# zipnn/zipnn

Measured on NVIDIA H100. Metric: compress+decompress GB/s on bf16 tensors, higher is better.
Workload: dtype u8

## Files before the change

zipnn_b200/csrc/api_compress.inc:

```

namespace {
struct EncWs {
  size_t part_off, part_bytes, types_off, sizes_off, itemoff_off, saves_off, hist_off, total;
};
inline EncWs enc_ws_layout(size_t n, int G, size_t chunk) {
  EncWs L;
  const uint64_t nitems = (uint64_t)G * num_chunks(n, chunk);
  L.part_off = kCtrlBytes;
  L.part_bytes = 8 * (size_t)G * ((num_chunks(n, chunk) + kScanItems - 1) / kScanItems);
  L.types_off = round_up(L.part_off + L.part_bytes, 256);
  L.sizes_off = round_up(L.types_off + nitems, 256);
  L.itemoff_off = round_up(L.sizes_off + 4 * nitems, 256);
  L.saves_off = round_up(L.itemoff_off + 8 * nitems, 256);
  L.hist_off = round_up(L.saves_off + sizeof(EncSave) * nitems, 256);
  L.total = L.hist_off + 2048 * nitems + 256;
  return L;
}

template <int G>
int launch_encode(const uint8_t* in, size_t n, uint32_t chunk, uint64_t K, int bits_mode, double thr, uint8_t* ws,
                  const EncWs& L, const void* h_hdr, uint32_t hdr_len, uint8_t* out, cudaStream_t st, void* h_total = nullptr,
                  cudaEvent_t len_ready = nullptr) {
  Ctrl* ctrl = (Ctrl*)ws;
  uint8_t* types = ws + L.types_off;
  uint32_t* sizes = (uint32_t*)(ws + L.sizes_off);
  uint64_t* item_off = (uint64_t*)(ws + L.itemoff_off);
  EncSave* saves = (EncSave*)(ws + L.saves_off);
  const int sms = sm_count_cached();
  uint16_t* hist = (uint16_t*)(ws + L.hist_off);
  ZB_CUDA(cudaMemsetAsync(ws, 0, L.types_off, st));
  {
    const size_t smem = sizeof(HistSmem<G>);
    if (smem > 48 * 1024 && !smem_attr(k_encode_hist<G>, smem)) return ZIPNN_B200_E_CUDA;
    const int blocks = (int)std::min<uint64_t>(K, (uint64_t)sms * resident_blocks(k_encode_hist<G>, smem, kEncThreads));
    ScopedTimer tm(kKEncodeStats, st);
    k_encode_hist<G><<<blocks, kEncThreads, smem, st>>>(in, n, chunk, K, bits_mode, hist);
    ZB_LAUNCHED();
  }
  {
    const size_t smem = sizeof(TableWarp) * kTableWarps;
    const uint64_t nitems = (uint64_t)G * K;
    const int blocks = (int)std::min<uint64_t>((nitems + kTableWarps - 1) / kTableWarps, (uint64_t)sms * 16);
    ScopedTimer tm(kKEncodeTable, st);
    k_encode_table<G><<<blocks, kTableWarps * 32, smem, st>>>(hist, n, chunk, K, thr, types, sizes, saves,
                                                              (unsigned long long*)(ws + L.part_off));
    ZB_LAUNCHED();
  }
  {
    ScopedTimer tm(kKEncodeScan, st);
    const unsigned nblk = (unsigned)((K + kScanItems - 1) / kScanItems);
    EncHeader hdr;
    memcpy(hdr.b, h_hdr, hdr_len);
    k_encode_scan<<<(unsigned)G * nblk, kScanThreads, 0, st>>>(sizes, types, G, K, hdr, hdr_len, out, item_off, ctrl,
                                                            (const unsigned long long*)(ws + L.part_off));
    ZB_LAUNCHED();
  }
  if (h_total) {
    ZB_CUDA(cudaMemcpyAsync(h_total, &ctrl->total_len, sizeof(uint64_t), cudaMemcpyDeviceToHost, st));
    ZB_CUDA(cudaEventRecord(len_ready, st));
  }
  if (chunk % (64u * G) != 0) {
    const int blocks = (int)std::min<uint64_t>((uint64_t)G * K, (uint64_t)sms * resident_blocks(k_encode_write<G>, 0, kEncThreads));
    ScopedTimer tm(kKEncodeWriteRagged, st);
    k_encode_write<G><<<blocks, kEncThreads, 0, st>>>(in, n, chunk, K, bits_mode, types, sizes, saves, item_off, out, 0);
    ZB_LAUNCHED();
    return ZIPNN_B200_OK;
  }
  {
    const int blocks = (int)std::min<uint64_t>(K, (uint64_t)sms * resident_blocks(k_encode_write_warp<G>, 0, kWbWarps * 32));
    ScopedTimer tm(kKEncodeWrite, st);
    k_encode_write_warp<G><<<blocks, kWbWarps * 32, 0, st>>>(in, n, chunk, K, bits_mode, types, sizes, saves, item_off, out);
    ZB_LAUNCHED();
  }
  if ((n % chunk) % (64u * G) != 0) {
    ScopedTimer tm(kKEncodeWriteRagged, st);
    k_encode_write<G><<<G, kEncThreads, 0, st>>>(in, n, chunk, K, bits_mode, types, sizes, saves, item_off, out, 1);
    ZB_LAUNCHED();
  }
  return ZIPNN_B200_OK;
}
}

extern "C" int zipnn_b200_compress_workspace_size(size_t n, int num_buf, size_t chunk, size_t* out) {
  if (!out || chunk == 0 || !(num_buf == 1 || num_buf == 2 || num_buf == 4)) return ZIPNN_B200_E_ARG;
  *out = enc_ws_layout(n, num_buf, chunk).total;
  return ZIPNN_B200_OK;
}

extern "C" int zipnn_b200_compress(const void* d_in, size_t n, const void* h_hdr, size_t hdr_len, int num_buf, int bits_mode,
                        int bytes_mode, size_t chunk, float threshold, void* d_out, size_t out_cap, size_t* out_len,
                        void* d_ws, size_t ws_bytes, void* cuda_stream) {
  if (!valid_layout(num_buf, bytes_mode, chunk)) return ZIPNN_B200_E_ARG;
  if (!h_hdr || hdr_len < 32 || hdr_len > kHdrMax || !d_out || !d_ws) return ZIPNN_B200_E_ARG;
  if (n && (!d_in || ((uintptr_t)d_in & 15))) return ZIPNN_B200_E_ARG;
  if ((uintptr_t)d_ws & 255) return ZIPNN_B200_E_ARG;
  size_t bound = 0;
  zipnn_b200_compress_bound(n, num_buf, chunk, hdr_len, &bound);
  if (out_cap < bound) return ZIPNN_B200_E_CAPACITY;
  cudaStream_t st = (cudaStream_t)cuda_stream;
  if (n == 0) {
    uint8_t tmp[kHdrMax];
    memcpy(tmp, h_hdr, hdr_len);
    const uint64_t t = hdr_len;
    memcpy(tmp + 24, &t, 8);
    ZB_CUDA(cudaMemcpyAsync(d_out, tmp, hdr_len, cudaMemcpyHostToDevice, st));
    ZB_CUDA(cudaStreamSynchronize(st));
    if (out_len) *out_len = hdr_len;
    return ZIPNN_B200_OK;
  }
  const EncWs L = enc_ws_layout(n, num_buf, chunk);
  if (ws_bytes < L.total) return ZIPNN_B200_E_CAPACITY;
  uint8_t* ws = (uint8_t*)d_ws;
  const uint64_t K = num_chunks(n, chunk);
  const double thr = (double)threshold;
  PinnedBlock total;
  WaitEvent len_ready;
  if (out_len && (!total.p || !len_ready.e)) return ZIPNN_B200_E_CUDA;
  const int rc = dispatch_G(num_buf, [&](auto g) -> int {
    return launch_encode<decltype(g)::value>((const uint8_t*)d_in, n, (uint32_t)chunk, K, bits_mode, thr, ws, L, h_hdr,
                                             (uint32_t)hdr_len, (uint8_t*)d_out, st, out_len ? total.p : nullptr, len_ready.e);
  });
  if (out_len) {
    const bool ok = cuda_ok(cudaEventSynchronize(len_ready.e));
    if (rc) return rc;
    if (!ok) return ZIPNN_B200_E_CUDA;
    uint64_t v = 0;
    memcpy(&v, total.p, sizeof(v));
    *out_len = (size_t)v;
  }
  return rc;
}

namespace {
static_assert(sizeof(size_t) == sizeof(uint64_t), "out_lens are filled by a strided copy of Ctrl::total_len");
constexpr int kEncBatchKernels = 5;
constexpr uint64_t kEncBatchMaxChunks = 16384;

uint64_t enc_batch_max_chunks() {
  const char* e = getenv("ZIPNN_B200_ENC_BATCH_MAX_CHUNKS");
  return e ? (uint64_t)atoll(e) : kEncBatchMaxChunks;
}

int check_compress_item(const zipnn_b200_compress_item& it) {
  if (!valid_layout(it.num_buf, it.bytes_mode, it.chunk)) return ZIPNN_B200_E_ARG;
  if (!it.h_hdr || it.hdr_len < 32 || it.hdr_len > kHdrMax || !it.d_out) return ZIPNN_B200_E_ARG;
  if (it.n && (!it.d_in || ((uintptr_t)it.d_in & 15))) return ZIPNN_B200_E_ARG;
  size_t bound = 0;
  zipnn_b200_compress_bound(it.n, it.num_buf, it.chunk, it.hdr_len, &bound);
  if (it.out_cap < bound) return ZIPNN_B200_E_CAPACITY;
  return ZIPNN_B200_OK;
}

inline int enc_class(int G) { return G == 1 ? 0 : (G == 2 ? 1 : 2); }

struct EncBatchLayout {
  std::vector<int> order;
  int cls_begin[4] = {0, 0, 0, 0};
  std::vector<uint64_t> starts;
  size_t start_at[3] = {0, 0, 0};
  std::vector<size_t> hdr_at, part_at, slice_at;
  std::vector<int> single;
  std::vector<char> one;
  size_t start_off = 0, hdr_off = 0, blob_bytes = 0, ctrl_off = 0, zero_bytes = 0, total = 0;
};

int enc_batch_layout(const zipnn_b200_compress_item* items, int n, EncBatchLayout& L) {
  if (n < 0 || (n && !items)) return ZIPNN_B200_E_ARG;
  for (int k = 0; k < 3; k++) {
    L.cls_begin[k] = (int)L.order.size();
    for (int i = 0; i < n; i++) {
      if (!(items[i].num_buf == 1 || items[i].num_buf == 2 || items[i].num_buf == 4)) return ZIPNN_B200_E_ARG;
      if (enc_class(items[i].num_buf) == k) L.order.push_back(i);
    }
  }
  L.cls_begin[3] = n;
  L.hdr_at.resize(n);
  L.part_at.resize(n);
  L.slice_at.resize(n);
  const uint64_t max_chunks = enc_batch_max_chunks();
  auto is_single = [&](int i) { return num_chunks(items[i].n, items[i].chunk) > max_chunks; };
  L.one.resize(n);
  for (int i = 0; i < n; i++)
    if ((L.one[i] = is_single(i))) L.single.push_back(i);
  for (int k = 0; k < 3; k++) {
    const int b = L.cls_begin[k], m = L.cls_begin[k + 1] - b;
    L.start_at[k] = L.starts.size();
    L.starts.resize(L.starts.size() + (size_t)kEncBatchKernels * (m + 1), 0);
    uint64_t* s = L.starts.data() + L.start_at[k];
    for (int j = 0; j < m; j++) {
      const zipnn_b200_compress_item& it = items[L.order[b + j]];
      const uint64_t G = (uint64_t)it.num_buf, K = num_chunks(it.n, it.chunk);
      const bool one = is_single(L.order[b + j]);
      const uint64_t work[kEncBatchKernels] = {
          K, G * K, K ? G * ((K + kScanItems - 1) / kScanItems) : 1, it.chunk % (64 * G) == 0 ? K : 0,
          it.chunk % (64 * G) != 0 ? G * K : ((it.n % it.chunk) % (64 * G) != 0 ? G : 0)};
      for (int q = 0; q < kEncBatchKernels; q++) s[q * (m + 1) + j + 1] = s[q * (m + 1) + j] + (one ? 0 : work[q]);
    }
    if (s[2 * (m + 1) + m] > 0x7fffffffull) return ZIPNN_B200_E_ARG;
  }
  L.start_off = round_up(sizeof(EncTensor) * (size_t)n, 256);
  L.hdr_off = round_up(L.start_off + sizeof(uint64_t) * L.starts.size(), 256);
  size_t at = L.hdr_off;
  for (int i = 0; i < n; i++) {
    L.hdr_at[i] = at;
    at += round_up(items[i].hdr_len, 16);
  }
  L.blob_bytes = at;
  L.ctrl_off = round_up(at, 256);
  at = L.ctrl_off + kCtrlBytes * (size_t)n;
  for (int i = 0; i < n; i++) {
    L.part_at[i] = at;
    at += items[i].n ? enc_ws_layout(items[i].n, items[i].num_buf, items[i].chunk).part_bytes : 0;
  }
  L.zero_bytes = at - L.ctrl_off;
  at = round_up(at, 256);
  for (int i = 0; i < n; i++) {
    L.slice_at[i] = at;
    if (items[i].n) {
      const EncWs W = enc_ws_layout(items[i].n, items[i].num_buf, items[i].chunk);
      at += round_up(is_single(i) ? W.total : W.total - W.types_off, 256);
    }
  }
  L.total = at;
  return ZIPNN_B200_OK;
}

template <int G>
int launch_encode_batch(const EncTensor* d_t, uint32_t m, const uint64_t* d_start, const uint64_t* h_start, cudaStream_t st) {
  auto batch = [&](int q) { EncBatch b; b.t = d_t; b.start = d_start + (size_t)q * (m + 1); b.n = m; return b; };
  auto total = [&](int q) { return h_start[(size_t)q * (m + 1) + m]; };
  const int sms = sm_count_cached();
  {
    const size_t smem = sizeof(HistSmem<G>);
    if (smem > 48 * 1024 && !smem_attr(k_encode_hist_batch<G>, smem)) return ZIPNN_B200_E_CUDA;
    const int per_sm = resident_blocks(k_encode_hist_batch<G>, smem, kEncThreads);
    const int blocks = (int)std::max<uint64_t>(1, std::min<uint64_t>(total(0), (uint64_t)sms * per_sm));
    ScopedTimer tm(kKEncodeStats, st);
    k_encode_hist_batch<G><<<blocks, kEncThreads, smem, st>>>(batch(0));
    ZB_LAUNCHED();
  }
  {
    const size_t smem = sizeof(TableWarp) * kTableWarps;
    const int blocks = (int)std::max<uint64_t>(1, std::min<uint64_t>((total(1) + kTableWarps - 1) / kTableWarps, (uint64_t)sms * 16));
    ScopedTimer tm(kKEncodeTable, st);
    k_encode_table_batch<G><<<blocks, kTableWarps * 32, smem, st>>>(batch(1));
    ZB_LAUNCHED();
  }
  {
    ScopedTimer tm(kKEncodeScan, st);
    k_encode_scan_batch<<<(unsigned)total(2), kScanThreads, 0, st>>>(batch(2));
    ZB_LAUNCHED();
  }
  {
    const int per_sm = resident_blocks(k_encode_write_warp<G, EncBatch>, 0, kWbWarps * 32);
    const int blocks = (int)std::max<uint64_t>(1, std::min<uint64_t>(total(3), (uint64_t)sms * per_sm));
    ScopedTimer tm(kKEncodeWrite, st);
    k_encode_write_warp<G, EncBatch><<<blocks, kWbWarps * 32, 0, st>>>(nullptr, 0, 0, 0, 0, nullptr, nullptr, nullptr, nullptr, nullptr, batch(3));
    ZB_LAUNCHED();
  }
  if (total(4)) {
    const int per_sm = resident_blocks(k_encode_write<G, EncBatch>, 0, kEncThreads);
    const int blocks = (int)std::min<uint64_t>(total(4), (uint64_t)sms * per_sm);
    ScopedTimer tm(kKEncodeWriteRagged, st);
    k_encode_write<G, EncBatch><<<blocks, kEncThreads, 0, st>>>(nullptr, 0, 0, 0, 0, nullptr, nullptr, nullptr, nullptr, nullptr, 0, batch(4));
    ZB_LAUNCHED();
  }
  return ZIPNN_B200_OK;
}
}

extern "C" int zipnn_b200_compress_batch_workspace_size(const zipnn_b200_compress_item* items, int n, size_t* out) {
  if (!out) return ZIPNN_B200_E_ARG;
  for (int i = 0; i < n && items; i++)
    if (!valid_layout(items[i].num_buf, items[i].bytes_mode, items[i].chunk)) return ZIPNN_B200_E_ARG;
  EncBatchLayout L;
  const int rc = enc_batch_layout(items, n, L);
  if (rc) return rc;
  *out = L.total;
  return ZIPNN_B200_OK;
}

extern "C" int zipnn_b200_compress_batch(const zipnn_b200_compress_item* items, int n, size_t* out_lens, void* d_ws, size_t ws_bytes,
                                         void* cuda_stream) {
  if (n < 0 || (n && !items)) return ZIPNN_B200_E_ARG;
  if (n == 0) return ZIPNN_B200_OK;
  if (!d_ws || ((uintptr_t)d_ws & 255)) return ZIPNN_B200_E_ARG;
  for (int i = 0; i < n; i++) {
    const int rc = check_compress_item(items[i]);
    if (rc) return rc;
  }
  EncBatchLayout L;
  {
    const int rc = enc_batch_layout(items, n, L);
    if (rc) return rc;
  }
  if (ws_bytes < L.total) return ZIPNN_B200_E_CAPACITY;
  uint8_t* ws = (uint8_t*)d_ws;
  std::vector<uint8_t> blob(L.blob_bytes, 0);
  EncTensor* T = reinterpret_cast<EncTensor*>(blob.data());
  for (int j = 0; j < n; j++) {
    const int i = L.order[j];
    const zipnn_b200_compress_item& it = items[i];
    const EncWs W = enc_ws_layout(it.n, it.num_buf, it.chunk);
    auto slice = [&](size_t off) { return ws + L.slice_at[i] + (off - (L.one[i] ? 0 : W.types_off)); };
    EncTensor& t = T[j];
    t.in = (const uint8_t*)it.d_in;
    t.out = (uint8_t*)it.d_out;
    t.hdr = ws + L.hdr_at[i];
    t.n = it.n;
    t.K = num_chunks(it.n, it.chunk);
    t.chunk = (uint32_t)it.chunk;
    t.hdr_len = (uint32_t)it.hdr_len;
    t.G = it.num_buf;
    t.bits_mode = it.bits_mode;
    t.thr = (double)it.threshold;
    t.ctrl = (Ctrl*)(ws + L.ctrl_off + kCtrlBytes * (size_t)i);
    t.partials = (unsigned long long*)(ws + L.part_at[i]);
    t.types = slice(W.types_off);
    t.sizes = (uint32_t*)slice(W.sizes_off);
    t.item_off = (uint64_t*)slice(W.itemoff_off);
    t.saves = (EncSave*)slice(W.saves_off);
    t.hist = (uint16_t*)slice(W.hist_off);
    memcpy(blob.data() + L.hdr_at[i], it.h_hdr, it.hdr_len);
  }
  memcpy(blob.data() + L.start_off, L.starts.data(), sizeof(uint64_t) * L.starts.size());
  cudaStream_t st = (cudaStream_t)cuda_stream;
  ZB_CUDA(cudaMemsetAsync(ws + L.ctrl_off, 0, L.zero_bytes, st));
  ZB_CUDA(cudaMemcpyAsync(ws, blob.data(), blob.size(), cudaMemcpyHostToDevice, st));
  for (int k = 0; k < 3; k++) {
    const uint32_t m = (uint32_t)(L.cls_begin[k + 1] - L.cls_begin[k]);
    if (m == 0 || L.starts[L.start_at[k] + 2 * (m + 1) + m] == 0) continue;
    const EncTensor* d_t = (const EncTensor*)ws + L.cls_begin[k];
    const uint64_t* d_start = (const uint64_t*)(ws + L.start_off) + L.start_at[k];
    const uint64_t* h_start = L.starts.data() + L.start_at[k];
    const int rc = dispatch_G(1 << k, [&](auto g) -> int { return launch_encode_batch<decltype(g)::value>(d_t, m, d_start, h_start, st); });
    if (rc) return rc;
  }
  for (int i : L.single) {
    const zipnn_b200_compress_item& it = items[i];
    const EncWs W = enc_ws_layout(it.n, it.num_buf, it.chunk);
    uint8_t* sws = ws + L.slice_at[i];
    const int rc = dispatch_G(it.num_buf, [&](auto g) -> int {
      return launch_encode<decltype(g)::value>((const uint8_t*)it.d_in, it.n, (uint32_t)it.chunk, num_chunks(it.n, it.chunk), it.bits_mode,
                                               (double)it.threshold, sws, W, it.h_hdr, (uint32_t)it.hdr_len, (uint8_t*)it.d_out, st);
    });
    if (rc) return rc;
    ZB_CUDA(cudaMemcpyAsync(ws + L.ctrl_off + kCtrlBytes * (size_t)i + offsetof(Ctrl, total_len), sws + offsetof(Ctrl, total_len),
                            sizeof(uint64_t), cudaMemcpyDeviceToDevice, st));
  }
  if (out_lens) {
    ZB_CUDA(cudaMemcpy2DAsync(out_lens, sizeof(size_t), ws + L.ctrl_off + offsetof(Ctrl, total_len), kCtrlBytes, sizeof(uint64_t),
                              (size_t)n, cudaMemcpyDeviceToHost, st));
    ZB_CUDA(cudaStreamSynchronize(st));
  }
  return ZIPNN_B200_OK;
}
```

zipnn_b200/csrc/encode.cuh:

```cuda
#pragma once
#include "common.cuh"
#include "stage1.cuh"

#include <type_traits>

namespace zb {

struct EncSave {
  uint8_t nb[256];
  uint8_t hdr[128];
  uint32_t hsize;
  uint32_t sbytes[4];
  uint32_t lg;
  uint32_t pad[2];
};
static_assert(sizeof(EncSave) == 416, "EncSave layout");

constexpr int kEncThreads = 256;

struct EncTensor {
  const uint8_t* in;
  uint8_t* out;
  const uint8_t* hdr;
  uint64_t n, K;
  uint32_t chunk, hdr_len;
  int G, bits_mode;
  double thr;
  Ctrl* ctrl;
  unsigned long long* partials;
  uint8_t* types;
  uint32_t* sizes;
  uint64_t* item_off;
  EncSave* saves;
  uint16_t* hist;
};

struct EncBatch {
  const EncTensor* t;
  const uint64_t* start;
  uint32_t n;
};
struct NoBatch {};
template <class Batch>
constexpr bool kIsBatch = !std::is_same<Batch, NoBatch>::value;
__device__ __forceinline__ uint64_t batch_work(NoBatch, uint64_t single) { return single; }
__device__ __forceinline__ uint64_t batch_work(const EncBatch& B, uint64_t) { return B.start[B.n]; }

template <int G>
__device__ __forceinline__ uint32_t rot_byte_at(const uint8_t* __restrict__ in_c, uint32_t chunk_len, uint32_t rot_words,
                                                uint32_t pos) {
  const uint32_t wi = pos >> 2;
  if (wi >= rot_words) return in_c[pos];
  (void)chunk_len;
  const uint32_t w = rot_word<G>(__ldg(reinterpret_cast<const uint32_t*>(in_c) + wi));
  return (w >> (8 * (pos & 3))) & 0xFFu;
}

template <int G>
struct HistCfg {
  static constexpr int R = (G == 4) ? 16 : 32;
  static constexpr int kShift = (G == 4) ? 6 : 7;
};

template <int G>
struct HistSmem {
  uint32_t rep[G][256][HistCfg<G>::R];
};

template <int G, class Batch>
__device__ __forceinline__ void encode_hist(const uint8_t* __restrict__ in, uint64_t n, uint32_t chunk, uint64_t K, int bits_mode,
                                            uint16_t* __restrict__ hist, Batch B) {
  extern __shared__ __align__(1024) unsigned char smem_raw[];
  HistSmem<G>& S = *reinterpret_cast<HistSmem<G>*>(smem_raw);
  constexpr int R = HistCfg<G>::R;
  const int tid = threadIdx.x, lane = tid & 31;
  const uint32_t col_bytes = (uint32_t)(lane % R) * 4;
  unsigned char* const col_p = reinterpret_cast<unsigned char*>(&S.rep[0][0][0]) + col_bytes;
  for (int i = tid; i < G * 256 * R; i += kEncThreads) (&S.rep[0][0][0])[i] = 0;
  __syncthreads();
  for (uint64_t w = blockIdx.x; w < batch_work(B, K); w += gridDim.x) {
    uint64_t c = w;
    if constexpr (kIsBatch<Batch>) {
      const uint32_t i = batch_find(B.start, B.n, w);
      const EncTensor& T = B.t[i];
      in = T.in; n = T.n; chunk = T.chunk; K = T.K; bits_mode = T.bits_mode; hist = T.hist;
      c = w - B.start[i];
    }
    const uint8_t* in_c = in + c * (uint64_t)chunk;
    const uint32_t chunk_len = (c == K - 1) ? (uint32_t)(n - c * (uint64_t)chunk) : chunk;
    const uint32_t rot_words = (bits_mode == 1 && G > 1) ? (chunk_len >> 2) : 0;
    const bool fast = (chunk_len % 64u) == 0;
    for (int q = 0; q < 4; q++) {
      const uint32_t inc = (q & 1) ? 0x10000u : 1u;
      if (fast) {
        const uint32_t qbytes = chunk_len >> 2;
        const uint4* src = reinterpret_cast<const uint4*>(in_c + (uint64_t)q * qbytes);
        const uint32_t nvec = qbytes >> 4;
        uint4 v[4], nv[4];
#pragma unroll
        for (int k = 0; k < 4; k++) {
          const uint32_t u = k * kEncThreads + tid;
          nv[k] = (u < nvec) ? __ldg(src + u) : make_uint4(0, 0, 0, 0);
        }
        for (uint32_t u0 = 0; u0 < nvec; u0 += 4 * kEncThreads) {
#pragma unroll
          for (int k = 0; k < 4; k++) v[k] = nv[k];
#pragma unroll
          for (int k = 0; k < 4; k++) {
            const uint32_t u = u0 + (4 + k) * kEncThreads + tid;
            if (u < nvec) nv[k] = __ldg(src + u);
          }
#pragma unroll
          for (int k = 0; k < 4; k++) {
            if (u0 + k * kEncThreads + tid < nvec) {
              uint32_t w[4] = {v[k].x, v[k].y, v[k].z, v[k].w};
#pragma unroll
              for (int i = 0; i < 4; i++) {
                if (rot_words) w[i] = rot_word<G>(w[i]);
#pragma unroll
                for (int b = 0; b < 4; b++) {
                  const uint32_t byte = __byte_perm(w[i], 0u, 0x4440u | (uint32_t)b);
                  atomicAdd(reinterpret_cast<uint32_t*>(col_p + ((4 * i + b) % G) * (256 * R * 4) + byte * (uint32_t)(R * 4)), inc);
                }
              }
            }
          }
        }
      } else {
        for (int g = 0; g < G; g++) {
          const uint32_t pl = plane_len(chunk_len, G, g);
          const uint32_t seg = (pl + 3) >> 2;
          const uint32_t j0 = min(pl, (uint32_t)q * seg), j1 = (q == 3) ? pl : min(pl, j0 + seg);
          for (uint32_t j = j0 + tid; j < j1; j += kEncThreads)
            atomicAdd(&S.rep[g][rot_byte_at<G>(in_c, chunk_len, rot_words, j * G + g)][lane % R], inc);
        }
      }
      if ((q & 1) == 0) continue;
      __syncthreads();
      for (int g = 0; g < G; g++) {
        uint32_t sum = 0;
#pragma unroll
        for (int r = 0; r < R; r++) {
          const int rr = (r + tid) % R;
          sum += S.rep[g][tid][rr];
          S.rep[g][tid][rr] = 0;
        }
        uint16_t* h = hist + (((uint64_t)g * K + c) * 4 + (q - 1)) * 256 + tid;
        h[0] = (uint16_t)(sum & 0xFFFFu);
        h[256] = (uint16_t)(sum >> 16);
      }
      __syncthreads();
    }
  }
}

template <int G>
__global__ void __launch_bounds__(kEncThreads) k_encode_hist(const uint8_t* __restrict__ in, uint64_t n, uint32_t chunk,
                                                             uint64_t K, int bits_mode, uint16_t* __restrict__ hist) {
  encode_hist<G>(in, n, chunk, K, bits_mode, hist, NoBatch{});
}

template <int G>
__global__ void __launch_bounds__(kEncThreads, G == 1 ? 2 : 3) k_encode_hist_batch(EncBatch B) {
  encode_hist<G>(nullptr, 0, 0, 0, 0, nullptr, B);
}

constexpr uint64_t kScanItems = 2048;

struct __align__(16) TableWarp {
  uint32_t total[256];
  uint8_t nb[256];
  uint8_t nzsym[256];
  TreeScratch tree;
};
constexpr int kTableWarps = 4;

__device__ void warp_block_decision(TableWarp& S, const uint16_t* __restrict__ hist, uint32_t plen, uint32_t cap, double thr,
                                    uint8_t* type_out, uint32_t* size_out, EncSave* save) {
  const int lane = threadIdx.x & 31;
  uint32_t* total = S.total;
  uint32_t largest = 0;
  int max_sym = -1;
  for (int s = lane; s < 256; s += 32) {
    const uint32_t t = (uint32_t)__ldg(hist + s) + __ldg(hist + 256 + s) + __ldg(hist + 512 + s) + __ldg(hist + 768 + s);
    total[s] = t;
    largest = max(largest, t);
    if (t) max_sym = s;
  }
#pragma unroll
  for (int o = 16; o; o >>= 1) {
    largest = max(largest, __shfl_xor_sync(0xffffffffu, largest, o));
    max_sym = max(max_sym, __shfl_xor_sync(0xffffffffu, max_sym, o));
  }
  __syncwarp();
  uint32_t stored = 0;
  const int early = huf_early_out(largest, plen);
  if (early == 1) {
    stored = huf_block_decision(true, nullptr, 0, plen, cap, thr);
    if (stored && lane == 0) {
      save->hdr[0] = (uint8_t)max_sym;
      save->hsize = 0;
    }
  }
  if (early == 2) {
    TreeScratch& T = S.tree;
    uint8_t* nz = S.nzsym;
    int k = 0;
    for (int base = 0; base < 256; base += 32) {
      const int s = base + lane;
      const bool p = total[s] != 0;
      const uint32_t m = __ballot_sync(0xffffffffu, p);
      if (p) nz[k + __popc(m & ((1u << lane) - 1u))] = (uint8_t)s;
      k += __popc(m);
    }
    __syncwarp();
    for (int i = lane; i < k; i += 32) {
      const uint32_t c = total[nz[i]];
      int rank = 0;
      for (int j = 0; j < k; j++) {
        const uint32_t cj = total[nz[j]];
        rank += (cj > c) || (cj == c && j < i);
      }
      T.cnt[rank] = c;
      T.sym[rank] = nz[i];
    }
    __syncwarp();
    int lg = 0, hsize = -1;
    if (lane == 0) {
      const int want = fse_pick_log(kHufLogDefault, plen, (uint32_t)max_sym, 1);
      lg = huf_lengths_from_sorted(T, k - 1, want, S.nb);
      hsize = huf_write_table(T, S.nb, max_sym, lg);
    }
    lg = __shfl_sync(0xffffffffu, lg, 0);
    hsize = __shfl_sync(0xffffffffu, hsize, 0);
    __syncwarp();
    if (hsize > 0 && (uint32_t)hsize + 12 < plen) {
      uint32_t bits[4] = {0, 0, 0, 0};
      for (int s = lane; s <= max_sym; s += 32) {
        const uint32_t l = S.nb[s];
#pragma unroll
        for (int q = 0; q < 4; q++) bits[q] += (uint32_t)__ldg(hist + 256 * q + s) * l;
      }
#pragma unroll
      for (int q = 0; q < 4; q++)
#pragma unroll
        for (int o = 16; o; o >>= 1) bits[q] += __shfl_xor_sync(0xffffffffu, bits[q], o);
      stored = huf_block_decision(false, bits, hsize, plen, cap, thr);
      if (stored) {
        for (int s = lane; s < 256; s += 32) save->nb[s] = S.nb[s];
        for (int i = lane; i < hsize; i += 32) save->hdr[i] = T.hdr[i];
        if (lane == 0) {
          save->hsize = (uint32_t)hsize;
          save->lg = (uint32_t)lg;
#pragma unroll
          for (int q = 0; q < 4; q++) save->sbytes[q] = (bits[q] >> 3) + 1;
        }
      }
    }
  }
  if (lane == 0) {
    *type_out = stored ? 1 : 0;
    *size_out = stored ? stored : plen;
  }
}

template <int G>
__device__ __forceinline__ void encode_table_item(TableWarp& S, const uint16_t* __restrict__ hist, uint64_t n, uint32_t chunk, uint64_t K,
                                                  double thr, uint8_t* types, uint32_t* sizes, EncSave* saves,
                                                  unsigned long long* partials, const int lane, uint64_t item) {
  {
    const int g = (int)(item / K);
    const uint64_t c = item - (uint64_t)g * K;
    const uint32_t chunk_len = (c == K - 1) ? (uint32_t)(n - c * (uint64_t)chunk) : chunk;
    warp_block_decision(S, hist + item * 1024, plane_len(chunk_len, G, g), chunk, thr, types + item, sizes + item, saves + item);
    __syncwarp();
    if (lane == 0) atomicAdd(partials + (uint64_t)g * ((K + kScanItems - 1) / kScanItems) + c / kScanItems, (unsigned long long)sizes[item]);
  }
}

template <int G>
__global__ void __launch_bounds__(kTableWarps * 32) k_encode_table(const uint16_t* __restrict__ hist, uint64_t n, uint32_t chunk,
                                                                   uint64_t K, double thr, uint8_t* types, uint32_t* sizes,
                                                                   EncSave* saves, unsigned long long* partials) {
  extern __shared__ __align__(1024) unsigned char smem_raw[];
  TableWarp& S = reinterpret_cast<TableWarp*>(smem_raw)[threadIdx.x >> 5];
  const int lane = threadIdx.x & 31;
  const uint64_t nitems = (uint64_t)G * K;
  for (uint64_t item = (uint64_t)blockIdx.x * kTableWarps + (threadIdx.x >> 5); item < nitems;
       item += (uint64_t)gridDim.x * kTableWarps)
    encode_table_item<G>(S, hist, n, chunk, K, thr, types, sizes, saves, partials, lane, item);
}

constexpr int kScanThreads = 256;

__device__ __forceinline__ void encode_scan_block(const uint32_t* __restrict__ sizes, const uint8_t* __restrict__ types, int G, uint64_t K,
                                                  const uint8_t* __restrict__ hdr_dev, uint32_t hdr_len, uint8_t* out, uint64_t* item_off,
                                                  Ctrl* ctrl, const unsigned long long* __restrict__ partials, uint32_t bid) {
  __shared__ uint64_t warp_tot[kScanThreads / 32];
  __shared__ uint64_t red[kScanThreads / 32][3];
  const int tid = threadIdx.x, lane = tid & 31, warp = tid >> 5;
  const uint64_t nitems = (uint64_t)G * K;
  const uint64_t nblk = (K + kScanItems - 1) / kScanItems;
  const int g = (int)(bid / nblk);
  const uint64_t blk = bid - (uint64_t)g * nblk;
  uint64_t s_groups = 0, s_blocks = 0, s_all = 0;
  for (uint64_t i = tid; i < (uint64_t)G * nblk; i += kScanThreads) {
    const uint64_t v = partials[i];
    const uint64_t gi = i / nblk;
    s_all += v;
    if (gi < (uint64_t)g) s_groups += v;
    if (gi == (uint64_t)g && i - gi * nblk < blk) s_blocks += v;
  }
#pragma unroll
  for (int o = 16; o; o >>= 1) {
    s_groups += __shfl_xor_sync(0xffffffffu, s_groups, o);
    s_blocks += __shfl_xor_sync(0xffffffffu, s_blocks, o);
    s_all += __shfl_xor_sync(0xffffffffu, s_all, o);
  }
  if (lane == 0) { red[warp][0] = s_groups; red[warp][1] = s_blocks; red[warp][2] = s_all; }
  __syncthreads();
  s_groups = s_blocks = s_all = 0;
  for (int w = 0; w < kScanThreads / 32; w++) { s_groups += red[w][0]; s_blocks += red[w][1]; s_all += red[w][2]; }
  const uint64_t payload0 = (uint64_t)hdr_len + 9 * nitems;
  const uint64_t base = payload0 + s_groups;
  const uint64_t c_first = blk * kScanItems + (uint64_t)tid * 8;
  uint32_t v[8];
  uint64_t run = 0;
#pragma unroll
  for (int j = 0; j < 8; j++) {
    v[j] = (c_first + j < K) ? sizes[(uint64_t)g * K + c_first + j] : 0u;
    run += v[j];
  }
  uint64_t x = run;
#pragma unroll
  for (int o = 1; o < 32; o <<= 1) {
    const uint64_t y = __shfl_up_sync(0xffffffffu, x, o);
    if (lane >= o) x += y;
  }
  if (lane == 31) warp_tot[warp] = x;
  __syncthreads();
  uint64_t pre = s_blocks + x - run;
  for (int w = 0; w < warp; w++) pre += warp_tot[w];
  uint8_t* cum_out = out + hdr_len + nitems;
#pragma unroll
  for (int j = 0; j < 8; j++) {
    const uint64_t c = c_first + j;
    if (c < K) {
      const uint64_t i = (uint64_t)g * K + c;
      item_off[i] = base + pre;
      pre += v[j];
      st_u64_bytes(cum_out + 8 * i, pre);
      out[hdr_len + i] = types[i];
    }
  }
  if (blk == 0 && tid == 0) {
    ctrl->base[g] = base;
    uint64_t tot = 0;
    for (uint64_t j = 0; j < nblk; j++) tot += partials[(uint64_t)g * nblk + j];
    ctrl->group_total[g] = tot;
  }
  if (bid == 0) {
    const uint64_t total = payload0 + s_all;
    for (uint32_t i = tid; i < hdr_len; i += kScanThreads) {
      uint8_t b = hdr_dev[i];
      if (i >= 24 && i < 32) b = (uint8_t)(total >> (8 * (i - 24)));
      out[i] = b;
    }
    if (tid == 0) ctrl->total_len = total;
  }
}

constexpr size_t kHdrMax = 4096;
struct EncHeader {
  uint8_t b[kHdrMax];
};

__global__ void __launch_bounds__(kScanThreads) k_encode_scan(const uint32_t* __restrict__ sizes, const uint8_t* __restrict__ types,
                                                              int G, uint64_t K, const __grid_constant__ EncHeader hdr,
                                                              uint32_t hdr_len, uint8_t* out, uint64_t* item_off, Ctrl* ctrl,
                                                              const unsigned long long* __restrict__ partials) {
  encode_scan_block(sizes, types, G, K, hdr.b, hdr_len, out, item_off, ctrl, partials, blockIdx.x);
}

constexpr uint32_t kEncTile = kEncThreads * 16;
constexpr uint32_t kBitBufWords = (kEncTile * 11) / 32 + 8;

struct WriteSmem {
  __align__(16) uint8_t tile[kEncTile + 16];
  uint32_t bitbuf[kBitBufWords];
  uint32_t code[256];
  uint32_t warp_sum[kEncThreads / 32];
  EncSave save;
};

template <int G>
__device__ __forceinline__ void stage_tile(uint8_t* tile, const uint8_t* __restrict__ in_c, uint32_t chunk_len,
                                           uint32_t rot_words, int g, uint32_t p0, uint32_t cnt) {
  const int tid = threadIdx.x;
  const bool fast = ((p0 * G) % 16u) == 0 && (cnt % 16u) == 0 && ((p0 + cnt) * (uint32_t)G <= (chunk_len & ~3u));
  if (fast) {
    for (uint32_t u = tid; u < (cnt >> 4); u += kEncThreads) {
      const uint4* src = reinterpret_cast<const uint4*>(in_c + (uint64_t)(p0 + 16 * u) * G);
      uint32_t w[4 * G];
#pragma unroll
      for (int i = 0; i < G; i++) {
        const uint4 v = __ldg(src + i);
        w[4 * i] = v.x; w[4 * i + 1] = v.y; w[4 * i + 2] = v.z; w[4 * i + 3] = v.w;
      }
      if (rot_words) {
#pragma unroll
        for (int i = 0; i < 4 * G; i++) w[i] = rot_word<G>(w[i]);
      }
      uint4 pv[G];
      split16<G>(w, pv);
      uint4 mine = pv[0];
#pragma unroll
      for (int k = 1; k < G; k++)
        if (g == k) mine = pv[k];
      *reinterpret_cast<uint4*>(tile + 16 * u) = mine;
    }
  } else {
    for (uint32_t j = tid; j < cnt; j += kEncThreads)
      tile[j] = (uint8_t)rot_byte_at<G>(in_c, chunk_len, rot_words, (p0 + j) * G + g);
  }
}

__device__ __forceinline__ void tile_to_global(const uint8_t* tile, uint8_t* dst, uint32_t cnt) {
  const int tid = threadIdx.x;
  const uint32_t head = min(cnt, (uint32_t)((16 - ((uintptr_t)dst & 15)) & 15));
  if ((uint32_t)tid < head) dst[tid] = tile[tid];
  const uint32_t nvec = (cnt - head) >> 4;
  const uint32_t* t32 = reinterpret_cast<const uint32_t*>(tile);
  for (uint32_t v = tid; v < nvec; v += kEncThreads) {
    const uint32_t o = head + 16 * v;
    const uint32_t sh = (o & 3) * 8;
    const uint32_t* p = t32 + (o >> 2);
    const uint32_t a0 = p[0], a1 = p[1], a2 = p[2], a3 = p[3], a4 = p[4];
    *reinterpret_cast<uint4*>(dst + o) = make_uint4(__funnelshift_r(a0, a1, sh), __funnelshift_r(a1, a2, sh),
                                                    __funnelshift_r(a2, a3, sh), __funnelshift_r(a3, a4, sh));
  }
  const uint32_t done = head + 16 * nvec;
  if ((uint32_t)tid < cnt - done) dst[done + tid] = tile[done + tid];
}

template <bool kValHigh>
__device__ __forceinline__ void warp_build_codes(const uint8_t* nb, int lg, uint32_t* code) {
  const int lane = threadIdx.x & 31;
  uint32_t per_len[kHufLogMax + 1];
#pragma unroll
  for (int l = 0; l <= kHufLogMax; l++) per_len[l] = 0;
  for (int base = 0; base < 256; base += 32) {
    const int mine = nb[base + lane];
#pragma unroll
    for (int l = 1; l <= kHufLogMax; l++) per_len[l] += __popc(__ballot_sync(0xffffffffu, mine == l));
  }
  uint32_t start[kHufLogMax + 1];
  {
    uint32_t v = 0;
#pragma unroll
    for (int l = kHufLogMax; l >= 1; l--) {
      if (l <= lg) {
        start[l] = v;
        v = (v + per_len[l]) >> 1;
      } else {
        start[l] = 0;
      }
    }
  }
  for (int base = 0; base < 256; base += 32) {
    const int mine = nb[base + lane];
    uint32_t val = 0;
#pragma unroll
    for (int l = 1; l <= kHufLogMax; l++) {
      const uint32_t m = __ballot_sync(0xffffffffu, mine == l);
      if (mine == l) val = start[l] + __popc(m & ((1u << lane) - 1u));
      start[l] += __popc(m);
    }
    code[base + lane] = kValHigh ? ((val << 8) | (uint32_t)mine) : (val | ((uint32_t)mine << 16));
  }
}

template <int G, class Batch = NoBatch>
__global__ void __launch_bounds__(kEncThreads) k_encode_write(const uint8_t* __restrict__ in, uint64_t n, uint32_t chunk, uint64_t K,
                                                              int bits_mode, const uint8_t* __restrict__ types,
                                                              const uint32_t* __restrict__ sizes, const EncSave* __restrict__ saves,
                                                              const uint64_t* __restrict__ item_off, uint8_t* out,
                                                              int only_ragged, Batch B = {}) {
  __shared__ WriteSmem S;
  const int tid = threadIdx.x, lane = tid & 31, warp = tid >> 5;
  const uint64_t nitems = (uint64_t)G * K;
  const uint64_t first = only_ragged ? (uint64_t)blockIdx.x * K + (K - 1) : blockIdx.x;
  const uint64_t step = only_ragged ? nitems : gridDim.x;
  for (uint64_t w = first; w < batch_work(B, nitems); w += step) {
    uint64_t item = w;
    if constexpr (kIsBatch<Batch>) {
      const uint32_t i = batch_find(B.start, B.n, w);
      const EncTensor& T = B.t[i];
      in = T.in; n = T.n; chunk = T.chunk; K = T.K; bits_mode = T.bits_mode;
      types = T.types; sizes = T.sizes; saves = T.saves; item_off = T.item_off; out = T.out;
      const uint64_t j = w - B.start[i];
      item = (chunk % (64u * G) != 0) ? j : j * K + (K - 1);
    }
    const int g = (int)(item / K);
    const uint64_t c = item - (uint64_t)g * K;
    const uint8_t* in_c = in + c * (uint64_t)chunk;
    const uint32_t chunk_len = (c == K - 1) ? (uint32_t)(n - c * (uint64_t)chunk) : chunk;
    if (only_ragged && chunk_len % (64u * G) == 0) continue;
    const uint32_t rot_words = (bits_mode == 1 && G > 1) ? (chunk_len >> 2) : 0;
    const uint32_t plen = plane_len(chunk_len, G, g);
    uint8_t* dest = out + item_off[item];
    const uint8_t type = types[item];
    const uint32_t size = sizes[item];
    if (plen == 0) continue;
    __syncthreads();
    if (type == 0) {
      for (uint32_t p0 = 0; p0 < plen; p0 += kEncTile) {
        const uint32_t cnt = min(kEncTile, plen - p0);
        stage_tile<G>(S.tile, in_c, chunk_len, rot_words, g, p0, cnt);
        __syncthreads();
        tile_to_global(S.tile, dest + p0, cnt);
        __syncthreads();
      }
      continue;
    }
    if (size == 1) {
      if (tid == 0) dest[0] = saves[item].hdr[0];
      continue;
    }
    {
      const uint32_t* sv = reinterpret_cast<const uint32_t*>(saves + item);
      uint32_t* dv = reinterpret_cast<uint32_t*>(&S.save);
      for (int i = tid; i < (int)(sizeof(EncSave) / 4); i += kEncThreads) dv[i] = sv[i];
    }
    __syncthreads();
    const uint32_t hsize = S.save.hsize;
    if (warp == 0) warp_build_codes<false>(S.save.nb, (int)S.save.lg, S.code);
    if (warp == 1) {
      for (uint32_t i = lane; i < hsize; i += 32) dest[i] = S.save.hdr[i];
      if (lane < 3) {
        dest[hsize + 2 * lane] = (uint8_t)S.save.sbytes[lane];
        dest[hsize + 2 * lane + 1] = (uint8_t)(S.save.sbytes[lane] >> 8);
      }
    }
    __syncthreads();
    const uint32_t seg = (plen + 3) >> 2;
    uint32_t stream_at = hsize + 6;
    for (int i = 0; i < 4; i++) {
      const uint32_t s_begin = (uint32_t)i * seg;
      const uint32_t s_end = (i == 3) ? plen : s_begin + seg;
      uint8_t* gaddr = dest + stream_at;
      const uint32_t sbytes = S.save.sbytes[i];
      stream_at += sbytes;
      const uint32_t a = (uint32_t)((uintptr_t)gaddr & 3);
      uint32_t* gword = reinterpret_cast<uint32_t*>(gaddr - a);
      uint32_t B = 8 * a;
      uint32_t flushed = 0;
      for (uint32_t w = tid; w < kBitBufWords; w += kEncThreads) S.bitbuf[w] = 0;
      __syncthreads();
      for (uint32_t p1 = s_end; p1 > s_begin;) {
        const uint32_t p0 = (p1 - s_begin > kEncTile) ? p1 - kEncTile : s_begin;
        const uint32_t cnt = p1 - p0;
        stage_tile<G>(S.tile, in_c, chunk_len, rot_words, g, p0, cnt);
        __syncthreads();
        const uint32_t e0 = 16u * tid;
        const int nvalid = (int)min(16u, cnt > e0 ? cnt - e0 : 0u);
        uint64_t v[4] = {0, 0, 0, 0};
        uint32_t l[4] = {0, 0, 0, 0};
        if (nvalid == 16 && (cnt & 15u) == 0) {
          const uint4 q = *reinterpret_cast<const uint4*>(S.tile + (cnt - 16 - e0));
          const uint32_t wv[4] = {q.x, q.y, q.z, q.w};
#pragma unroll
          for (int k = 0; k < 16; k++) {
            const uint32_t sym = (wv[(15 - k) >> 2] >> (8 * ((15 - k) & 3))) & 0xFFu;
            const uint32_t cd = S.code[sym];
            v[k >> 2] |= (uint64_t)(cd & 0xFFFFu) << l[k >> 2];
            l[k >> 2] += cd >> 16;
          }
        } else {
          for (int k = 0; k < nvalid; k++) {
            const uint32_t cd = S.code[S.tile[cnt - 1 - (e0 + k)]];
            v[k >> 2] |= (uint64_t)(cd & 0xFFFFu) << l[k >> 2];
            l[k >> 2] += cd >> 16;
          }
        }
        const uint32_t mine = l[0] + l[1] + l[2] + l[3];
        uint32_t x = mine;
#pragma unroll
        for (int o = 1; o < 32; o <<= 1) {
          const uint32_t y = __shfl_up_sync(0xffffffffu, x, o);
          if (lane >= o) x += y;
        }
        if (lane == 31) S.warp_sum[warp] = x;
        __syncthreads();
        uint32_t pre = 0, tile_bits = 0;
#pragma unroll
        for (int w = 0; w < kEncThreads / 32; w++) {
          const uint32_t t = S.warp_sum[w];
          if (w < warp) pre += t;
          tile_bits += t;
        }
        uint32_t off = (B - 32 * flushed) + pre + x - mine;
#pragma unroll
        for (int r = 0; r < 4; r++) {
          if (l[r]) {
            const uint32_t sh = off & 31, wi = off >> 5;
            const uint32_t lo32 = (uint32_t)v[r], hi32 = (uint32_t)(v[r] >> 32);
            const uint32_t w0 = lo32 << sh;
            const uint32_t w1 = __funnelshift_l(lo32, hi32, sh);
            const uint32_t w2 = sh ? (hi32 >> (32 - sh)) : 0u;
            if (w0) atomicOr(&S.bitbuf[wi], w0);
            if (w1) atomicOr(&S.bitbuf[wi + 1], w1);
            if (w2) atomicOr(&S.bitbuf[wi + 2], w2);
            off += l[r];
          }
        }
        __syncthreads();
        B += tile_bits;
        const uint32_t complete = (B >> 5) - flushed;
        for (uint32_t w = tid; w < complete; w += kEncThreads) {
          const uint32_t val = S.bitbuf[w];
          if (flushed + w == 0 && a != 0) {
            for (uint32_t bb = a; bb < 4; bb++) gaddr[bb - a] = (uint8_t)(val >> (8 * bb));
          } else {
            gword[flushed + w] = val;
          }
        }
        const uint32_t carry = S.bitbuf[complete];
        __syncthreads();
        for (uint32_t w = tid; w <= complete + 1 && w < kBitBufWords; w += kEncThreads) S.bitbuf[w] = 0;
        __syncthreads();
        if (tid == 0) S.bitbuf[0] = carry;
        flushed += complete;
        p1 = p0;
        __syncthreads();
      }
      if (tid == 0) S.bitbuf[(B - 32 * flushed) >> 5] |= 1u << (B & 31);
      __syncthreads();
      {
        const uint32_t first_byte = max(4 * flushed, a);
        const uint32_t end_byte = a + sbytes;
        for (uint32_t bb = first_byte + tid; bb < end_byte; bb += kEncThreads) {
          const uint32_t rel = bb - 4 * flushed;
          gaddr[bb - a] = (uint8_t)(S.bitbuf[rel >> 2] >> (8 * (rel & 3)));
        }
      }
      __syncthreads();
    }
  }
}

constexpr int kWbWarps = 4;
constexpr uint32_t kWbTile = 512;
constexpr uint32_t kWbBitWords = (kWbTile * 11) / 32 + 4;

__device__ __forceinline__ void rotate_planes(uint32_t& lo, uint32_t& hi) {
  const uint32_t l = lo, h = hi;
  hi = ((h << 1) & 0xFEFEFEFEu) | ((l >> 7) & 0x01010101u);
  lo = (h & 0x80808080u) | (l & 0x7F7F7F7Fu);
}

struct WbItem {
  uint8_t* dest;
  uint32_t size;
  uint32_t hsize;
  uint32_t sbytes[4];
  uint32_t lg;
  uint32_t type;
};

template <int G>
struct WbSmem {
  uint32_t code[G][256];
  WbItem item[G];
  __align__(16) uint8_t nb[G][256];
  uint32_t bitbuf[kWbWarps][G][kWbBitWords];
  __align__(16) uint8_t stage[kWbWarps][kWbTile + 32];
};

struct WbStream {
  uint8_t* gaddr;
  uint32_t a;
  uint32_t B;
  uint32_t flushed;
};

__device__ __forceinline__ void wb_flush(uint32_t* bitbuf, WbStream& st, int lane) {
  uint32_t* gword = reinterpret_cast<uint32_t*>(st.gaddr - st.a);
  const uint32_t complete = (st.B >> 5) - st.flushed;
  const bool split_first = (st.flushed == 0 && st.a != 0);
  if (split_first && lane == 0 && complete > 0) {
    const uint32_t val = bitbuf[0];
    for (uint32_t bb = st.a; bb < 4; bb++) st.gaddr[bb - st.a] = (uint8_t)(val >> (8 * bb));
  }
  for (uint32_t w = lane; w < complete; w += 32) {
    const uint32_t val = bitbuf[w];
    bitbuf[w] = 0;
    if (!(split_first && w == 0)) gword[st.flushed + w] = val;
  }
  if (lane == 0 && complete > 0) {
    bitbuf[0] = bitbuf[complete];
    bitbuf[complete] = 0;
  }
  st.flushed += complete;
  __syncwarp();
}

template <int G, class Batch = NoBatch>
__global__ void __launch_bounds__(kWbWarps * 32) k_encode_write_warp(const uint8_t* __restrict__ in, uint64_t n, uint32_t chunk,
                                                                     uint64_t K, int bits_mode, const uint8_t* __restrict__ types,
                                                                     const uint32_t* __restrict__ sizes,
                                                                     const EncSave* __restrict__ saves,
                                                                     const uint64_t* __restrict__ item_off, uint8_t* out,
                                                                     Batch B = {}) {
  __shared__ WbSmem<G> S;
  const int tid = threadIdx.x, lane = tid & 31, warp = tid >> 5;
  for (uint64_t w = blockIdx.x; w < batch_work(B, K); w += gridDim.x) {
    uint64_t c = w;
    if constexpr (kIsBatch<Batch>) {
      const uint32_t i = batch_find(B.start, B.n, w);
      const EncTensor& T = B.t[i];
      in = T.in; n = T.n; chunk = T.chunk; K = T.K; bits_mode = T.bits_mode;
      types = T.types; sizes = T.sizes; saves = T.saves; item_off = T.item_off; out = T.out;
      c = w - B.start[i];
    }
    const uint32_t chunk_len = (c == K - 1) ? (uint32_t)(n - c * (uint64_t)chunk) : chunk;
    if (chunk_len % (64u * G) != 0) continue;
    const uint8_t* in_c = in + c * (uint64_t)chunk;
    const uint32_t plen = chunk_len / G;
    const uint32_t seg = plen >> 2;
    const bool rot = (bits_mode == 1 && G > 1);
    __syncthreads();
    if (warp < G) {
      const int g = warp;
      const uint64_t item = (uint64_t)g * K + c;
      WbItem it;
      it.dest = out + item_off[item];
      it.type = types[item];
      it.size = sizes[item];
      it.hsize = 0;
      it.lg = 0;
      it.sbytes[0] = it.sbytes[1] = it.sbytes[2] = it.sbytes[3] = 0;
      if (it.type == 1 && it.size == 1) {
        if (lane == 0) it.dest[0] = saves[item].hdr[0];
      } else if (it.type == 1) {
        const EncSave* sv = saves + item;
        it.hsize = sv->hsize;
        it.lg = sv->lg;
#pragma unroll
        for (int q = 0; q < 4; q++) it.sbytes[q] = sv->sbytes[q];
        reinterpret_cast<uint2*>(S.nb[g])[lane] = reinterpret_cast<const uint2*>(sv->nb)[lane];
        __syncwarp();
        warp_build_codes<true>(S.nb[g], (int)it.lg, S.code[g]);
        for (uint32_t i = lane; i < it.hsize; i += 32) it.dest[i] = sv->hdr[i];
        if (lane < 3) {
          it.dest[it.hsize + 2 * lane] = (uint8_t)it.sbytes[lane];
          it.dest[it.hsize + 2 * lane + 1] = (uint8_t)(it.sbytes[lane] >> 8);
        }
      }
      if (lane == 0) S.item[g] = it;
    }
    __syncthreads();

    const int s = warp;
    WbStream st[G];
    uint32_t raw_shift[G];
#pragma unroll
    for (int g = 0; g < G; g++) {
      const WbItem& it = S.item[g];
      st[g].gaddr = it.dest;
      st[g].a = st[g].B = st[g].flushed = 0;
      raw_shift[g] = 0;
      if (it.type == 1 && it.size > 1) {
        uint32_t at = it.hsize + 6;
        for (int q = 0; q < s; q++) at += it.sbytes[q];
        st[g].gaddr = it.dest + at;
        st[g].a = (uint32_t)((uintptr_t)st[g].gaddr & 3);
        st[g].B = 8 * st[g].a;
        for (uint32_t w = lane; w < kWbBitWords; w += 32) S.bitbuf[warp][g][w] = 0;
      } else if (it.type == 0) {
        st[g].gaddr = it.dest + (uint64_t)s * seg;
        raw_shift[g] = (uint32_t)((uintptr_t)st[g].gaddr & 15);
      }
    }
    __syncwarp();

    const uint8_t* src_s = in_c + (uint64_t)s * seg * G;
    const uint32_t ntiles = (seg + kWbTile - 1) / kWbTile;
    uint4 cur[G], nxt[G];
    {
      const uint32_t t0 = (ntiles - 1) * kWbTile;
      if (t0 + 16 * lane < seg) {
        const uint4* p = reinterpret_cast<const uint4*>(src_s + (uint64_t)(t0 + 16 * lane) * G);
#pragma unroll
        for (int i = 0; i < G; i++) nxt[i] = __ldg(p + i);
      }
    }
    auto do_tile = [&](auto full_tag, const uint32_t ti) {
      constexpr bool kFull = decltype(full_tag)::value;
      const uint32_t t0 = ti * kWbTile;
      const uint32_t cnt = kFull ? kWbTile : min(kWbTile, seg - t0);
      const bool have = kFull ? true : (16u * lane < cnt);
#pragma unroll
      for (int i = 0; i < G; i++) cur[i] = nxt[i];
      if (ti > 0) {
        const uint4* p = reinterpret_cast<const uint4*>(src_s + (uint64_t)(t0 - kWbTile + 16 * lane) * G);
#pragma unroll
        for (int i = 0; i < G; i++) nxt[i] = __ldg(p + i);
      }
      uint4 pv[G];
      if (have) {
        uint32_t w[4 * G];
#pragma unroll
        for (int i = 0; i < G; i++) {
          w[4 * i] = cur[i].x; w[4 * i + 1] = cur[i].y; w[4 * i + 2] = cur[i].z; w[4 * i + 3] = cur[i].w;
        }
        split16<G>(w, pv);
        if (rot) {
          rotate_planes(pv[(G - 2) % G].x, pv[G - 1].x);
          rotate_planes(pv[(G - 2) % G].y, pv[G - 1].y);
          rotate_planes(pv[(G - 2) % G].z, pv[G - 1].z);
          rotate_planes(pv[(G - 2) % G].w, pv[G - 1].w);
        }
      }
#pragma unroll
      for (int g = 0; g < G; g++) {
        const uint32_t type = S.item[g].type, size = S.item[g].size;
        if (type == 0) {
          uint8_t* stg = S.stage[warp];
          if (have) *reinterpret_cast<uint4*>(stg + 16 * lane) = pv[g];
          __syncwarp();
          uint8_t* D = st[g].gaddr + t0;
          const uint32_t m = raw_shift[g];
          if (m == 0) {
            if (have) *reinterpret_cast<uint4*>(D + 16 * lane) = pv[g];
          } else {
            const uint32_t head = 16 - m;
            const uint32_t nblk = (cnt - head) >> 4;
            {
              const uint4 a4 = *reinterpret_cast<const uint4*>(stg + 16 * lane);
              const uint4 b4 = *reinterpret_cast<const uint4*>(stg + 16 * lane + 16);
              const uint32_t wv[8] = {a4.x, a4.y, a4.z, a4.w, b4.x, b4.y, b4.z, b4.w};
              const uint32_t bs = (head & 3) * 8;
              uint32_t o[4];
              switch (head >> 2) {
                case 0:
#pragma unroll
                  for (int i = 0; i < 4; i++) o[i] = __funnelshift_r(wv[i], wv[i + 1], bs);
                  break;
                case 1:
#pragma unroll
                  for (int i = 0; i < 4; i++) o[i] = __funnelshift_r(wv[i + 1], wv[i + 2], bs);
                  break;
                case 2:
#pragma unroll
                  for (int i = 0; i < 4; i++) o[i] = __funnelshift_r(wv[i + 2], wv[i + 3], bs);
                  break;
                default:
#pragma unroll
                  for (int i = 0; i < 4; i++) o[i] = __funnelshift_r(wv[i + 3], wv[i + 4], bs);
                  break;
              }
              if ((uint32_t)lane < nblk) *reinterpret_cast<uint4*>(D + head + 16 * lane) = make_uint4(o[0], o[1], o[2], o[3]);
            }
            if (kFull) {
              if (lane < 16) {
                const uint32_t idx = (uint32_t)lane < head ? (uint32_t)lane : (kWbTile - 16u + (uint32_t)lane);
                D[idx] = stg[idx];
              }
            } else {
              if ((uint32_t)lane < head) D[lane] = stg[lane];
              const uint32_t done = head + 16 * nblk;
              if ((uint32_t)lane < cnt - done) D[done + lane] = stg[done + lane];
            }
          }
          __syncwarp();
        } else if (size > 1) {
          const unsigned char* code = reinterpret_cast<const unsigned char*>(S.code[g]);
          uint64_t v[4] = {0, 0, 0, 0};
          uint32_t l[4] = {0, 0, 0, 0};
          if (have) {
            const uint32_t wv[4] = {pv[g].x, pv[g].y, pv[g].z, pv[g].w};
#pragma unroll
            for (int r = 0; r < 4; r++) {
              const uint32_t w = wv[3 - r];
              const uint32_t e3 = *reinterpret_cast<const uint32_t*>(code + ((w >> 22) & 0x3FCu));
              const uint32_t e2 = *reinterpret_cast<const uint32_t*>(code + ((w >> 14) & 0x3FCu));
              const uint32_t e1 = *reinterpret_cast<const uint32_t*>(code + ((w >> 6) & 0x3FCu));
              const uint32_t e0 = *reinterpret_cast<const uint32_t*>(code + ((w << 2) & 0x3FCu));
              const uint32_t n3 = e3 & 0xFFu, n2 = e2 & 0xFFu, n1 = e1 & 0xFFu, n0 = e0 & 0xFFu;
              const uint32_t hi = (e3 >> 8) | ((e2 >> 8) << n3);
              const uint32_t lo = (e1 >> 8) | ((e0 >> 8) << n1);
              const uint32_t lh = n3 + n2;
              v[r] = (uint64_t)hi | ((uint64_t)lo << lh);
              l[r] = lh + n1 + n0;
            }
          }
          const uint32_t mine = l[0] + l[1] + l[2] + l[3];
          uint32_t x = mine;
#pragma unroll
          for (int o = 1; o < 32; o <<= 1) {
            const uint32_t y = __shfl_down_sync(0xffffffffu, x, o);
            if (lane + o < 32) x += y;
          }
          const uint32_t tile_bits = __shfl_sync(0xffffffffu, x, 0);
          uint32_t* bitbuf = S.bitbuf[warp][g];
          uint32_t off = (st[g].B - 32 * st[g].flushed) + (x - mine);
          const uint32_t bitbuf_s = (uint32_t)__cvta_generic_to_shared(bitbuf);
#pragma unroll
          for (int r = 0; r < 4; r++) {
            const uint32_t sh = off & 31, sa = bitbuf_s + ((off >> 5) << 2);
            const uint32_t lo32 = (uint32_t)v[r], hi32 = (uint32_t)(v[r] >> 32);
            const uint32_t w0 = lo32 << sh;
            const uint32_t w1 = __funnelshift_l(lo32, hi32, sh);
            const uint32_t w2 = (hi32 >> 1) >> (31 - sh);
            asm volatile("red.shared.or.b32 [%0], %1;" ::"r"(sa), "r"(w0) : "memory");
            asm volatile("red.shared.or.b32 [%0+4], %1;" ::"r"(sa), "r"(w1) : "memory");
            asm volatile("{ .reg .pred p; setp.ne.u32 p, %1, 0; @p red.shared.or.b32 [%0+8], %1; }" ::"r"(sa), "r"(w2) : "memory");
            off += l[r];
          }
          __syncwarp();
          st[g].B += tile_bits;
          wb_flush(bitbuf, st[g], lane);
        }
      }
        };
    do_tile(std::false_type{}, ntiles - 1);
    for (uint32_t ti = ntiles - 1; ti-- > 0;) do_tile(std::true_type{}, ti);
#pragma unroll
    for (int g = 0; g < G; g++) {
      if (S.item[g].type == 1 && S.item[g].size > 1) {
        uint32_t* bitbuf = S.bitbuf[warp][g];
        if (lane == 0) bitbuf[(st[g].B - 32 * st[g].flushed) >> 5] |= 1u << (st[g].B & 31);
        __syncwarp();
        const uint32_t first_byte = max(4 * st[g].flushed, st[g].a);
        const uint32_t end_byte = st[g].a + S.item[g].sbytes[s];
        for (uint32_t bb = first_byte + lane; bb < end_byte; bb += 32) {
          const uint32_t rel = bb - 4 * st[g].flushed;
          st[g].gaddr[bb - st[g].a] = (uint8_t)(bitbuf[rel >> 2] >> (8 * (rel & 3)));
        }
        __syncwarp();
      }
    }
  }
}

template <int G>
__global__ void __launch_bounds__(kTableWarps * 32) k_encode_table_batch(EncBatch B) {
  extern __shared__ __align__(1024) unsigned char smem_raw[];
  TableWarp& S = reinterpret_cast<TableWarp*>(smem_raw)[threadIdx.x >> 5];
  const int lane = threadIdx.x & 31;
  const uint64_t total = B.start[B.n];
  for (uint64_t w = (uint64_t)blockIdx.x * kTableWarps + (threadIdx.x >> 5); w < total; w += (uint64_t)gridDim.x * kTableWarps) {
    const uint32_t i = batch_find(B.start, B.n, w);
    const EncTensor& T = B.t[i];
    encode_table_item<G>(S, T.hist, T.n, T.chunk, T.K, T.thr, T.types, T.sizes, T.saves, T.partials, lane, w - B.start[i]);
  }
}

__global__ void __launch_bounds__(kScanThreads) k_encode_scan_batch(EncBatch B) {
  const uint32_t i = batch_find(B.start, B.n, blockIdx.x);
  const EncTensor& T = B.t[i];
  if (T.K == 0) {
    for (uint32_t j = threadIdx.x; j < T.hdr_len; j += kScanThreads)
      T.out[j] = (j >= 24 && j < 32) ? (uint8_t)((uint64_t)T.hdr_len >> (8 * (j - 24))) : T.hdr[j];
    if (threadIdx.x == 0) T.ctrl->total_len = T.hdr_len;
    return;
  }
  encode_scan_block(T.sizes, T.types, T.G, T.K, T.hdr, T.hdr_len, T.out, T.item_off, T.ctrl, T.partials,
                    (uint32_t)(blockIdx.x - B.start[i]));
}

}
```

Before: 544.5.

## Prebuild Huffman codes in table pass and pipeline warp write with dynamic claims

Builds canonical Huffman code words once in the table kernel and stores them in EncSave, so the write kernels no longer rebuild codes per item. Moves the header and stream-size emission into the scan kernel. Restructures the warp write kernel into per-warp units claimed through an atomic work counter, double-buffering unit metadata and codes with cp.async so the next unit's fetch overlaps the current unit's coding. Adds an optional phase-timing and emit-ceiling probe under a compile flag. In exchange EncSave grows from 416 to 1184 bytes per item, and the per-warp double-buffered shared memory can lower occupancy.

```diff
diff --git a/zipnn_b200/csrc/api_compress.inc b/zipnn_b200/csrc/api_compress.inc
--- a/zipnn_b200/csrc/api_compress.inc
+++ b/zipnn_b200/csrc/api_compress.inc
@@ -51,7 +51,7 @@
     const unsigned nblk = (unsigned)((K + kScanItems - 1) / kScanItems);
     EncHeader hdr;
     memcpy(hdr.b, h_hdr, hdr_len);
-    k_encode_scan<<<(unsigned)G * nblk, kScanThreads, 0, st>>>(sizes, types, G, K, hdr, hdr_len, out, item_off, ctrl,
+    k_encode_scan<<<(unsigned)G * nblk, kScanThreads, 0, st>>>(sizes, types, saves, G, K, hdr, hdr_len, out, item_off, ctrl,
                                                             (const unsigned long long*)(ws + L.part_off));
     ZB_LAUNCHED();
   }
@@ -69,7 +69,8 @@
   {
     const int blocks = (int)std::min<uint64_t>(K, (uint64_t)sms * resident_blocks(k_encode_write_warp<G>, 0, kWbWarps * 32));
     ScopedTimer tm(kKEncodeWrite, st);
-    k_encode_write_warp<G><<<blocks, kWbWarps * 32, 0, st>>>(in, n, chunk, K, bits_mode, types, sizes, saves, item_off, out);
+    k_encode_write_warp<G><<<blocks, kWbWarps * 32, 0, st>>>(in, n, chunk, K, bits_mode, types, sizes, saves, item_off, out,
+                                                               &ctrl->work_counter);
     ZB_LAUNCHED();
   }
   if ((n % chunk) % (64u * G) != 0) {
@@ -255,7 +256,7 @@
     const int per_sm = resident_blocks(k_encode_write_warp<G, EncBatch>, 0, kWbWarps * 32);
     const int blocks = (int)std::max<uint64_t>(1, std::min<uint64_t>(total(3), (uint64_t)sms * per_sm));
     ScopedTimer tm(kKEncodeWrite, st);
-    k_encode_write_warp<G, EncBatch><<<blocks, kWbWarps * 32, 0, st>>>(nullptr, 0, 0, 0, 0, nullptr, nullptr, nullptr, nullptr, nullptr, batch(3));
+    k_encode_write_warp<G, EncBatch><<<blocks, kWbWarps * 32, 0, st>>>(nullptr, 0, 0, 0, 0, nullptr, nullptr, nullptr, nullptr, nullptr, nullptr, batch(3));
     ZB_LAUNCHED();
   }
   if (total(4)) {
@@ -355,3 +356,34 @@
   }
   return ZIPNN_B200_OK;
 }
+
+#ifdef ZB_EMIT_PHASES
+extern "C" int zipnn_b200_emit_phases_read(unsigned long long* out, int reset) {
+  if (!out) return ZIPNN_B200_E_ARG;
+  ZB_CUDA(cudaMemcpyFromSymbol(out, g_emit_phases, sizeof(g_emit_phases)));
+  if (reset) {
+    const unsigned long long zero[kPhCount] = {};
+    ZB_CUDA(cudaMemcpyToSymbol(g_emit_phases, zero, sizeof(zero)));
+  }
+  return ZIPNN_B200_OK;
+}
+
+extern "C" int zipnn_b200_emit_ceiling(const void* d_in, size_t n, int num_buf, size_t chunk, void* d_ws, void* d_out, void* cuda_stream) {
+  if (!d_in || !d_ws || !d_out || n == 0 || !(num_buf == 1 || num_buf == 2 || num_buf == 4) || chunk % (64u * num_buf) != 0)
+    return ZIPNN_B200_E_ARG;
+  const EncWs L = enc_ws_layout(n, num_buf, chunk);
+  uint8_t* ws = (uint8_t*)d_ws;
+  uint32_t* claim = &((Ctrl*)ws)->work_counter;
+  const uint64_t K = num_chunks(n, chunk);
+  cudaStream_t st = (cudaStream_t)cuda_stream;
+  ZB_CUDA(cudaMemsetAsync(claim, 0, sizeof(uint32_t), st));
+  return dispatch_G(num_buf, [&](auto g) -> int {
+    constexpr int G = decltype(g)::value;
+    const int blocks = (int)std::min<uint64_t>(K, (uint64_t)sm_count_cached() * resident_blocks(k_encode_write_warp<G>, 0, kWbWarps * 32));
+    k_emit_ceiling<G><<<blocks, kWbWarps * 32, 0, st>>>((const uint8_t*)d_in, n, (uint32_t)chunk, K, (const uint32_t*)(ws + L.sizes_off),
+                                                        (const uint64_t*)(ws + L.itemoff_off), (uint8_t*)d_out, claim);
+    ZB_CUDA(cudaGetLastError());
+    return ZIPNN_B200_OK;
+  });
+}
+#endif
diff --git a/zipnn_b200/csrc/encode.cuh b/zipnn_b200/csrc/encode.cuh
--- a/zipnn_b200/csrc/encode.cuh
+++ b/zipnn_b200/csrc/encode.cuh
@@ -2,19 +2,21 @@
 #include "common.cuh"
 #include "stage1.cuh"
 
+#include <cstddef>
 #include <type_traits>
 
 namespace zb {
 
 struct EncSave {
-  uint8_t nb[256];
+  uint32_t code[256];
   uint8_t hdr[128];
+  uint32_t sbytes[4];
   uint32_t hsize;
-  uint32_t sbytes[4];
-  uint32_t lg;
-  uint32_t pad[2];
-};
-static_assert(sizeof(EncSave) == 416, "EncSave layout");
+  uint32_t pad[3];
+};
+static_assert(sizeof(EncSave) == 1184 && sizeof(EncSave) % 16 == 0, "EncSave layout");
+static_assert(offsetof(EncSave, code) == 0 && offsetof(EncSave, hdr) == 1024 && offsetof(EncSave, sbytes) == 1152 &&
+              offsetof(EncSave, hsize) == 1168, "EncSave layout: code and sbytes are copied in 16-byte pieces");
 
 constexpr int kEncThreads = 256;
 
@@ -175,6 +177,42 @@
 };
 constexpr int kTableWarps = 4;
 
+__device__ __forceinline__ void warp_build_codes(const uint8_t* nb, int lg, uint32_t* code) {
+  const int lane = threadIdx.x & 31;
+  uint32_t per_len[kHufLogMax + 1];
+#pragma unroll
+  for (int l = 0; l <= kHufLogMax; l++) per_len[l] = 0;
+  for (int base = 0; base < 256; base += 32) {
+    const int mine = nb[base + lane];
+#pragma unroll
+    for (int l = 1; l <= kHufLogMax; l++) per_len[l] += __popc(__ballot_sync(0xffffffffu, mine == l));
+  }
+  uint32_t start[kHufLogMax + 1];
+  {
+    uint32_t v = 0;
+#pragma unroll
+    for (int l = kHufLogMax; l >= 1; l--) {
+      if (l <= lg) {
+        start[l] = v;
+        v = (v + per_len[l]) >> 1;
+      } else {
+        start[l] = 0;
+      }
+    }
+  }
+  for (int base = 0; base < 256; base += 32) {
+    const int mine = nb[base + lane];
+    uint32_t val = 0;
+#pragma unroll
+    for (int l = 1; l <= kHufLogMax; l++) {
+      const uint32_t m = __ballot_sync(0xffffffffu, mine == l);
+      if (mine == l) val = start[l] + __popc(m & ((1u << lane) - 1u));
+      start[l] += __popc(m);
+    }
+    code[base + lane] = (val << 8) | (uint32_t)mine;
+  }
+}
+
 __device__ void warp_block_decision(TableWarp& S, const uint16_t* __restrict__ hist, uint32_t plen, uint32_t cap, double thr,
                                     uint8_t* type_out, uint32_t* size_out, EncSave* save) {
   const int lane = threadIdx.x & 31;
@@ -247,11 +285,10 @@
         for (int o = 16; o; o >>= 1) bits[q] += __shfl_xor_sync(0xffffffffu, bits[q], o);
       stored = huf_block_decision(false, bits, hsize, plen, cap, thr);
       if (stored) {
-        for (int s = lane; s < 256; s += 32) save->nb[s] = S.nb[s];
+        warp_build_codes(S.nb, lg, save->code);
         for (int i = lane; i < hsize; i += 32) save->hdr[i] = T.hdr[i];
         if (lane == 0) {
           save->hsize = (uint32_t)hsize;
-          save->lg = (uint32_t)lg;
 #pragma unroll
           for (int q = 0; q < 4; q++) save->sbytes[q] = (bits[q] >> 3) + 1;
         }
@@ -293,7 +330,8 @@
 
 constexpr int kScanThreads = 256;
 
-__device__ __forceinline__ void encode_scan_block(const uint32_t* __restrict__ sizes, const uint8_t* __restrict__ types, int G, uint64_t K,
+__device__ __forceinline__ void encode_scan_block(const uint32_t* __restrict__ sizes, const uint8_t* __restrict__ types,
+                                                  const EncSave* __restrict__ saves, int G, uint64_t K,
                                                   const uint8_t* __restrict__ hdr_dev, uint32_t hdr_len, uint8_t* out, uint64_t* item_off,
                                                   Ctrl* ctrl, const unsigned long long* __restrict__ partials, uint32_t bid) {
   __shared__ uint64_t warp_tot[kScanThreads / 32];
@@ -353,6 +391,47 @@
       out[hdr_len + i] = types[i];
     }
   }
+  __syncthreads();
+  {
+    const uint64_t c_hi = min(K, (blk + 1) * kScanItems);
+    for (uint64_t c0 = blk * kScanItems + (uint64_t)warp * 16; c0 < c_hi; c0 += (kScanThreads / 32) * 16) {
+      const uint64_t i0 = (uint64_t)g * K + c0;
+      const uint32_t nk = (uint32_t)min((uint64_t)16, c_hi - c0);
+      uint32_t ty = 0, sz = 0, hs = 0, sb[3] = {0, 0, 0};
+      uint64_t off = 0;
+      if ((uint32_t)lane < nk) {
+        const uint64_t i = i0 + lane;
+        ty = types[i];
+        sz = sizes[i];
+        off = item_off[i];
+        hs = saves[i].hsize;
+#pragma unroll
+        for (int q = 0; q < 3; q++) sb[q] = saves[i].sbytes[q];
+      }
+      uint32_t hw[16];
+#pragma unroll
+      for (int k = 0; k < 16; k++) hw[k] = ((uint32_t)k < nk) ? reinterpret_cast<const uint32_t*>(saves[i0 + k].hdr)[lane] : 0u;
+#pragma unroll
+      for (int k = 0; k < 16; k++) {
+        const uint32_t t = __shfl_sync(0xffffffffu, ty, k), z = __shfl_sync(0xffffffffu, sz, k);
+        const uint32_t h = __shfl_sync(0xffffffffu, hs, k);
+        const uint32_t j0 = __shfl_sync(0xffffffffu, sb[0], k), j1 = __shfl_sync(0xffffffffu, sb[1], k);
+        const uint32_t j2 = __shfl_sync(0xffffffffu, sb[2], k);
+        const uint32_t jump = lane < 2 ? j0 : (lane < 4 ? j1 : j2);
+        const uint64_t o = __shfl_sync(0xffffffffu, off, k);
+        if ((uint32_t)k >= nk || t != 1) continue;
+        uint8_t* d = out + o;
+        if (z == 1) {
+          if (lane == 0) d[0] = (uint8_t)hw[k];
+          continue;
+        }
+#pragma unroll
+        for (int b = 0; b < 4; b++)
+          if (4u * lane + b < h) d[4 * lane + b] = (uint8_t)(hw[k] >> (8 * b));
+        if (lane < 6) d[h + lane] = (uint8_t)(jump >> (8 * (lane & 1)));
+      }
+    }
+  }
   if (blk == 0 && tid == 0) {
     ctrl->base[g] = base;
     uint64_t tot = 0;
@@ -376,10 +455,10 @@
 };
 
 __global__ void __launch_bounds__(kScanThreads) k_encode_scan(const uint32_t* __restrict__ sizes, const uint8_t* __restrict__ types,
-                                                              int G, uint64_t K, const __grid_constant__ EncHeader hdr,
+                                                              const EncSave* __restrict__ saves, int G, uint64_t K, const __grid_constant__ EncHeader hdr,
                                                               uint32_t hdr_len, uint8_t* out, uint64_t* item_off, Ctrl* ctrl,
                                                               const unsigned long long* __restrict__ partials) {
-  encode_scan_block(sizes, types, G, K, hdr.b, hdr_len, out, item_off, ctrl, partials, blockIdx.x);
+  encode_scan_block(sizes, types, saves, G, K, hdr.b, hdr_len, out, item_off, ctrl, partials, blockIdx.x);
 }
 
 constexpr uint32_t kEncTile = kEncThreads * 16;
@@ -390,8 +469,10 @@
   uint32_t bitbuf[kBitBufWords];
   uint32_t code[256];
   uint32_t warp_sum[kEncThreads / 32];
-  EncSave save;
-};
+  uint32_t sbytes[4];
+  uint32_t hsize;
+};
+static_assert(kEncThreads == 256, "k_encode_write: one code word per thread");
 
 template <int G>
 __device__ __forceinline__ void stage_tile(uint8_t* tile, const uint8_t* __restrict__ in_c, uint32_t chunk_len,
@@ -441,43 +522,6 @@
   }
   const uint32_t done = head + 16 * nvec;
   if ((uint32_t)tid < cnt - done) dst[done + tid] = tile[done + tid];
-}
-
-template <bool kValHigh>
-__device__ __forceinline__ void warp_build_codes(const uint8_t* nb, int lg, uint32_t* code) {
-  const int lane = threadIdx.x & 31;
-  uint32_t per_len[kHufLogMax + 1];
-#pragma unroll
-  for (int l = 0; l <= kHufLogMax; l++) per_len[l] = 0;
-  for (int base = 0; base < 256; base += 32) {
-    const int mine = nb[base + lane];
-#pragma unroll
-    for (int l = 1; l <= kHufLogMax; l++) per_len[l] += __popc(__ballot_sync(0xffffffffu, mine == l));
-  }
-  uint32_t start[kHufLogMax + 1];
-  {
-    uint32_t v = 0;
-#pragma unroll
-    for (int l = kHufLogMax; l >= 1; l--) {
-      if (l <= lg) {
-        start[l] = v;
-        v = (v + per_len[l]) >> 1;
-      } else {
-        start[l] = 0;
-      }
-    }
-  }
-  for (int base = 0; base < 256; base += 32) {
-    const int mine = nb[base + lane];
-    uint32_t val = 0;
-#pragma unroll
-    for (int l = 1; l <= kHufLogMax; l++) {
-      const uint32_t m = __ballot_sync(0xffffffffu, mine == l);
-      if (mine == l) val = start[l] + __popc(m & ((1u << lane) - 1u));
-      start[l] += __popc(m);
-    }
-    code[base + lane] = kValHigh ? ((val << 8) | (uint32_t)mine) : (val | ((uint32_t)mine << 16));
-  }
 }
 
 template <int G, class Batch = NoBatch>
@@ -523,33 +567,23 @@
       }
       continue;
     }
-    if (size == 1) {
-      if (tid == 0) dest[0] = saves[item].hdr[0];
-      continue;
-    }
+    if (size == 1) continue;
     {
-      const uint32_t* sv = reinterpret_cast<const uint32_t*>(saves + item);
-      uint32_t* dv = reinterpret_cast<uint32_t*>(&S.save);
-      for (int i = tid; i < (int)(sizeof(EncSave) / 4); i += kEncThreads) dv[i] = sv[i];
+      const EncSave& sv = saves[item];
+      const uint32_t e = sv.code[tid];
+      S.code[tid] = (e >> 8) | ((e & 0xFFu) << 16);
+      if (tid < 4) S.sbytes[tid] = sv.sbytes[tid];
+      if (tid == 0) S.hsize = sv.hsize;
     }
     __syncthreads();
-    const uint32_t hsize = S.save.hsize;
-    if (warp == 0) warp_build_codes<false>(S.save.nb, (int)S.save.lg, S.code);
-    if (warp == 1) {
-      for (uint32_t i = lane; i < hsize; i += 32) dest[i] = S.save.hdr[i];
-      if (lane < 3) {
-        dest[hsize + 2 * lane] = (uint8_t)S.save.sbytes[lane];
-        dest[hsize + 2 * lane + 1] = (uint8_t)(S.save.sbytes[lane] >> 8);
-      }
-    }
-    __syncthreads();
+    const uint32_t hsize = S.hsize;
     const uint32_t seg = (plen + 3) >> 2;
     uint32_t stream_at = hsize + 6;
     for (int i = 0; i < 4; i++) {
       const uint32_t s_begin = (uint32_t)i * seg;
       const uint32_t s_end = (i == 3) ? plen : s_begin + seg;
       uint8_t* gaddr = dest + stream_at;
-      const uint32_t sbytes = S.save.sbytes[i];
+      const uint32_t sbytes = S.sbytes[i];
       stream_at += sbytes;
       const uint32_t a = (uint32_t)((uintptr_t)gaddr & 3);
       uint32_t* gword = reinterpret_cast<uint32_t*>(gaddr - a);
@@ -659,23 +693,85 @@
   lo = (h & 0x80808080u) | (l & 0x7F7F7F7Fu);
 }
 
-struct WbItem {
-  uint8_t* dest;
-  uint32_t size;
-  uint32_t hsize;
-  uint32_t sbytes[4];
-  uint32_t lg;
-  uint32_t type;
+enum : uint32_t { kWbRaw = 0, kWbCoded = 1, kWbNone = 2 };
+
+template <int G>
+struct WbUnit {
+  const uint8_t* src;
+  uint8_t* dest[G];
+  uint32_t kind[G];
+  uint32_t sbytes[G];
+  uint32_t seg;
+  uint32_t rot;
+};
+
+struct __align__(16) WbFetch {
+  uint32_t sbytes[4][4];
+  uint64_t off[4];
+  uint32_t size[4];
+  uint32_t type4[4];
+  uint32_t hsize[4];
+  uint8_t* out;
+  const EncSave* save_c;
+  uint64_t K;
+  uint32_t item0;
+  uint32_t s;
 };
 
 template <int G>
 struct WbSmem {
-  uint32_t code[G][256];
-  WbItem item[G];
-  __align__(16) uint8_t nb[G][256];
+  uint32_t code[kWbWarps][2][G][256];
+  WbUnit<G> unit[kWbWarps][2];
+  WbFetch fetch[kWbWarps];
   uint32_t bitbuf[kWbWarps][G][kWbBitWords];
   __align__(16) uint8_t stage[kWbWarps][kWbTile + 32];
 };
+
+__device__ __forceinline__ void wb_cp_async(void* smem_dst, const void* gmem_src, int bytes) {
+  const uint32_t d = (uint32_t)__cvta_generic_to_shared(smem_dst);
+  if (bytes == 16) asm volatile("cp.async.cg.shared.global [%0], [%1], 16;\n" ::"r"(d), "l"(gmem_src) : "memory");
+  else if (bytes == 8) asm volatile("cp.async.ca.shared.global [%0], [%1], 8;\n" ::"r"(d), "l"(gmem_src) : "memory");
+  else asm volatile("cp.async.ca.shared.global [%0], [%1], 4;\n" ::"r"(d), "l"(gmem_src) : "memory");
+}
+__device__ __forceinline__ void wb_cp_async_wait() {
+  asm volatile("cp.async.commit_group;\ncp.async.wait_group 0;\n" ::: "memory");
+}
+
+enum : int { kPhSetup = 0, kPhWait = 1, kPhCode = 2, kPhTail = 3, kPhCount = 4 };
+#ifdef ZB_EMIT_PHASES
+__device__ unsigned long long g_emit_phases[kPhCount];
+struct PhaseClock {
+  long long last, acc[kPhCount];
+  __device__ __forceinline__ PhaseClock() {
+    last = clock64();
+#pragma unroll
+    for (int p = 0; p < kPhCount; p++) acc[p] = 0;
+  }
+  __device__ __forceinline__ void mark(int p) {
+    const long long t = clock64();
+    acc[p] += t - last;
+    last = t;
+  }
+  template <int N>
+  __device__ __forceinline__ void wait_for(const uint4 (&v)[N]) {
+#pragma unroll
+    for (int i = 0; i < N; i++) asm volatile("" ::"r"(v[i].x));
+    mark(kPhWait);
+  }
+  __device__ __forceinline__ void commit(int lane) {
+    if (lane == 0)
+#pragma unroll
+      for (int p = 0; p < kPhCount; p++) atomicAdd(&g_emit_phases[p], (unsigned long long)acc[p]);
+  }
+};
+#else
+struct PhaseClock {
+  __device__ __forceinline__ void mark(int) {}
+  template <int N>
+  __device__ __forceinline__ void wait_for(const uint4 (&)[N]) {}
+  __device__ __forceinline__ void commit(int) {}
+};
+#endif
 
 struct WbStream {
   uint8_t* gaddr;
@@ -705,16 +801,13 @@
   __syncwarp();
 }
 
-template <int G, class Batch = NoBatch>
-__global__ void __launch_bounds__(kWbWarps * 32) k_encode_write_warp(const uint8_t* __restrict__ in, uint64_t n, uint32_t chunk,
-                                                                     uint64_t K, int bits_mode, const uint8_t* __restrict__ types,
-                                                                     const uint32_t* __restrict__ sizes,
-                                                                     const EncSave* __restrict__ saves,
-                                                                     const uint64_t* __restrict__ item_off, uint8_t* out,
-                                                                     Batch B = {}) {
-  __shared__ WbSmem<G> S;
-  const int tid = threadIdx.x, lane = tid & 31, warp = tid >> 5;
-  for (uint64_t w = blockIdx.x; w < batch_work(B, K); w += gridDim.x) {
+template <int G, class Batch>
+__device__ __forceinline__ void wb_fetch_items(WbUnit<G>& U, WbFetch& F, uint64_t u, uint64_t units, const uint8_t* in, uint64_t n,
+                                               uint32_t chunk, uint64_t K, int bits_mode, const uint8_t* types, const uint32_t* sizes,
+                                               const EncSave* saves, const uint64_t* item_off, uint8_t* out, const Batch& B, int lane) {
+  uint32_t seg = 0;
+  if (u < units) {
+    const uint64_t w = u >> 2;
     uint64_t c = w;
     if constexpr (kIsBatch<Batch>) {
       const uint32_t i = batch_find(B.start, B.n, w);
@@ -724,77 +817,140 @@
       c = w - B.start[i];
     }
     const uint32_t chunk_len = (c == K - 1) ? (uint32_t)(n - c * (uint64_t)chunk) : chunk;
-    if (chunk_len % (64u * G) != 0) continue;
-    const uint8_t* in_c = in + c * (uint64_t)chunk;
-    const uint32_t plen = chunk_len / G;
-    const uint32_t seg = plen >> 2;
-    const bool rot = (bits_mode == 1 && G > 1);
-    __syncthreads();
-    if (warp < G) {
-      const int g = warp;
-      const uint64_t item = (uint64_t)g * K + c;
-      WbItem it;
-      it.dest = out + item_off[item];
-      it.type = types[item];
-      it.size = sizes[item];
-      it.hsize = 0;
-      it.lg = 0;
-      it.sbytes[0] = it.sbytes[1] = it.sbytes[2] = it.sbytes[3] = 0;
-      if (it.type == 1 && it.size == 1) {
-        if (lane == 0) it.dest[0] = saves[item].hdr[0];
-      } else if (it.type == 1) {
-        const EncSave* sv = saves + item;
-        it.hsize = sv->hsize;
-        it.lg = sv->lg;
-#pragma unroll
-        for (int q = 0; q < 4; q++) it.sbytes[q] = sv->sbytes[q];
-        reinterpret_cast<uint2*>(S.nb[g])[lane] = reinterpret_cast<const uint2*>(sv->nb)[lane];
-        __syncwarp();
-        warp_build_codes<true>(S.nb[g], (int)it.lg, S.code[g]);
-        for (uint32_t i = lane; i < it.hsize; i += 32) it.dest[i] = sv->hdr[i];
-        if (lane < 3) {
-          it.dest[it.hsize + 2 * lane] = (uint8_t)it.sbytes[lane];
-          it.dest[it.hsize + 2 * lane + 1] = (uint8_t)(it.sbytes[lane] >> 8);
-        }
-      }
-      if (lane == 0) S.item[g] = it;
-    }
-    __syncthreads();
-
-    const int s = warp;
+    if (chunk_len % (64u * G) == 0) {
+      const uint32_t s = (uint32_t)(u & 3);
+      seg = chunk_len / G / 4;
+      if (lane == 0) {
+        U.src = in + c * (uint64_t)chunk + (uint64_t)s * seg * G;
+        U.rot = (bits_mode == 1 && G > 1);
+        F.out = out;
+        F.save_c = saves + c;
+        F.K = K;
+        F.item0 = (uint32_t)(c & 3);
+        F.s = s;
+      }
+      const int g = lane & 7;
+      if (g < G) {
+        const uint64_t item = (uint64_t)g * K + c;
+        switch (lane >> 3) {
+          case 0: wb_cp_async(&F.off[g], item_off + item, 8); break;
+          case 1: wb_cp_async(&F.size[g], sizes + item, 4); break;
+          case 2: wb_cp_async(&F.type4[g], types + (item & ~(uint64_t)3), 4); break;
+          default:
+            wb_cp_async(F.sbytes[g], saves[item].sbytes, 16);
+            wb_cp_async(&F.hsize[g], &saves[item].hsize, 4);
+            break;
+        }
+      }
+    }
+  }
+  if (lane == 0) {
+    U.seg = seg;
+    if (seg == 0)
+#pragma unroll
+      for (int g = 0; g < G; g++) U.kind[g] = kWbNone;
+  }
+}
+
+template <int G>
+__device__ __forceinline__ void wb_fetch_codes(WbUnit<G>& U, const WbFetch& F, uint32_t (*code)[256], int lane) {
+  wb_cp_async_wait();
+  __syncwarp();
+  const uint32_t seg = U.seg;
+  if (seg == 0) return;
+#pragma unroll
+  for (int g = 0; g < G; g++) {
+    const uint64_t item_lo = (uint64_t)g * F.K + F.item0;
+    const uint32_t type = (F.type4[g] >> (8 * (uint32_t)(item_lo & 3))) & 0xFFu;
+    const uint32_t kind = type == 0 ? kWbRaw : (F.size[g] > 1 ? kWbCoded : kWbNone);
+    uint8_t* dest = F.out + F.off[g];
+    if (kind == kWbRaw) {
+      dest += (uint64_t)F.s * seg;
+    } else if (kind == kWbCoded) {
+      uint32_t at = F.hsize[g] + 6;
+      for (uint32_t q = 0; q < F.s; q++) at += F.sbytes[g][q];
+      dest += at;
+      const uint4* src = reinterpret_cast<const uint4*>(F.save_c[(uint64_t)g * F.K].code);
+      wb_cp_async(reinterpret_cast<uint4*>(code[g]) + lane, src + lane, 16);
+      wb_cp_async(reinterpret_cast<uint4*>(code[g]) + 32 + lane, src + 32 + lane, 16);
+    }
+    if (lane == 0) {
+      U.dest[g] = dest;
+      U.kind[g] = kind;
+      U.sbytes[g] = F.sbytes[g][F.s];
+    }
+  }
+  asm volatile("cp.async.commit_group;\n" ::: "memory");
+  __syncwarp();
+}
+
+template <int G, class Batch = NoBatch>
+__global__ void __launch_bounds__(kWbWarps * 32) k_encode_write_warp(const uint8_t* __restrict__ in, uint64_t n, uint32_t chunk,
+                                                                     uint64_t K, int bits_mode, const uint8_t* __restrict__ types,
+                                                                     const uint32_t* __restrict__ sizes,
+                                                                     const EncSave* __restrict__ saves,
+                                                                     const uint64_t* __restrict__ item_off, uint8_t* out,
+                                                                     uint32_t* claim, Batch B = {}) {
+  __shared__ WbSmem<G> S;
+  const int lane = threadIdx.x & 31, warp = threadIdx.x >> 5;
+  PhaseClock ph;
+  const uint64_t units = 4 * batch_work(B, K);
+  auto next_unit = [&]() -> uint64_t {
+    uint32_t v = 0;
+    if constexpr (kIsBatch<Batch>) {
+      if (lane == 0) v = atomicAdd(&B.t[0].ctrl->work_counter, 1u);
+    } else {
+      if (lane == 0) v = atomicAdd(claim, 1u);
+    }
+    return __shfl_sync(0xffffffffu, v, 0);
+  };
+  auto fetch_items = [&](int b, uint64_t v) {
+    wb_fetch_items<G>(S.unit[warp][b], S.fetch[warp], v, units, in, n, chunk, K, bits_mode, types, sizes, saves, item_off, out, B, lane);
+  };
+  auto fetch_codes = [&](int b) { wb_fetch_codes<G>(S.unit[warp][b], S.fetch[warp], S.code[warp][b], lane); };
+  uint4 cur[G], nxt[G];
+  auto load_first_tile = [&](int b) {
+    const WbUnit<G>& V = S.unit[warp][b];
+    const uint32_t t0 = ((V.seg + kWbTile - 1) / kWbTile - 1) * kWbTile;
+    if (V.seg && t0 + 16 * lane < V.seg) {
+      const uint4* p = reinterpret_cast<const uint4*>(V.src + (uint64_t)(t0 + 16 * lane) * G);
+#pragma unroll
+      for (int i = 0; i < G; i++) nxt[i] = __ldg(p + i);
+    }
+  };
+
+  uint64_t u = next_unit();
+  int b = 0;
+  fetch_items(0, u);
+  fetch_codes(0);
+  load_first_tile(0);
+  wb_cp_async_wait();
+  __syncwarp();
+  while (u < units) {
+    const uint64_t u_next = next_unit();
+    const WbUnit<G>& U = S.unit[warp][b];
+    const uint32_t seg = U.seg;
+    const uint8_t* const src_s = U.src;
+    const bool rot = U.rot;
     WbStream st[G];
     uint32_t raw_shift[G];
 #pragma unroll
     for (int g = 0; g < G; g++) {
-      const WbItem& it = S.item[g];
-      st[g].gaddr = it.dest;
+      st[g].gaddr = U.dest[g];
       st[g].a = st[g].B = st[g].flushed = 0;
       raw_shift[g] = 0;
-      if (it.type == 1 && it.size > 1) {
-        uint32_t at = it.hsize + 6;
-        for (int q = 0; q < s; q++) at += it.sbytes[q];
-        st[g].gaddr = it.dest + at;
+      if (U.kind[g] == kWbCoded) {
         st[g].a = (uint32_t)((uintptr_t)st[g].gaddr & 3);
         st[g].B = 8 * st[g].a;
         for (uint32_t w = lane; w < kWbBitWords; w += 32) S.bitbuf[warp][g][w] = 0;
-      } else if (it.type == 0) {
-        st[g].gaddr = it.dest + (uint64_t)s * seg;
+      } else if (U.kind[g] == kWbRaw) {
         raw_shift[g] = (uint32_t)((uintptr_t)st[g].gaddr & 15);
       }
     }
     __syncwarp();
-
-    const uint8_t* src_s = in_c + (uint64_t)s * seg * G;
+    ph.mark(kPhSetup);
+
     const uint32_t ntiles = (seg + kWbTile - 1) / kWbTile;
-    uint4 cur[G], nxt[G];
-    {
-      const uint32_t t0 = (ntiles - 1) * kWbTile;
-      if (t0 + 16 * lane < seg) {
-        const uint4* p = reinterpret_cast<const uint4*>(src_s + (uint64_t)(t0 + 16 * lane) * G);
-#pragma unroll
-        for (int i = 0; i < G; i++) nxt[i] = __ldg(p + i);
-      }
-    }
     auto do_tile = [&](auto full_tag, const uint32_t ti) {
       constexpr bool kFull = decltype(full_tag)::value;
       const uint32_t t0 = ti * kWbTile;
@@ -806,7 +962,10 @@
         const uint4* p = reinterpret_cast<const uint4*>(src_s + (uint64_t)(t0 - kWbTile + 16 * lane) * G);
 #pragma unroll
         for (int i = 0; i < G; i++) nxt[i] = __ldg(p + i);
-      }
+      } else {
+        load_first_tile(b ^ 1);
+      }
+      if (have) ph.wait_for(cur);
       uint4 pv[G];
       if (have) {
         uint32_t w[4 * G];
@@ -824,8 +983,8 @@
       }
 #pragma unroll
       for (int g = 0; g < G; g++) {
-        const uint32_t type = S.item[g].type, size = S.item[g].size;
-        if (type == 0) {
+        const uint32_t kind = U.kind[g];
+        if (kind == kWbRaw) {
           uint8_t* stg = S.stage[warp];
           if (have) *reinterpret_cast<uint4*>(stg + 16 * lane) = pv[g];
           __syncwarp();
@@ -874,8 +1033,8 @@
             }
           }
           __syncwarp();
-        } else if (size > 1) {
-          const unsigned char* code = reinterpret_cast<const unsigned char*>(S.code[g]);
+        } else if (kind == kWbCoded) {
+          const unsigned char* code = reinterpret_cast<const unsigned char*>(S.code[warp][b][g]);
           uint64_t v[4] = {0, 0, 0, 0};
           uint32_t l[4] = {0, 0, 0, 0};
           if (have) {
@@ -923,17 +1082,32 @@
           wb_flush(bitbuf, st[g], lane);
         }
       }
-        };
-    do_tile(std::false_type{}, ntiles - 1);
-    for (uint32_t ti = ntiles - 1; ti-- > 0;) do_tile(std::true_type{}, ti);
+      ph.mark(kPhCode);
+    };
+    if (ntiles <= 1) {
+      fetch_items(b ^ 1, u_next);
+      fetch_codes(b ^ 1);
+      ph.mark(kPhSetup);
+    }
+    if (ntiles > 0) do_tile(std::false_type{}, ntiles - 1);
+    else load_first_tile(b ^ 1);
+    if (ntiles > 1) {
+      fetch_items(b ^ 1, u_next);
+      ph.mark(kPhSetup);
+      const uint32_t h = (ntiles - 1) / 2;
+      for (uint32_t ti = ntiles - 1; ti-- > h;) do_tile(std::true_type{}, ti);
+      fetch_codes(b ^ 1);
+      ph.mark(kPhSetup);
+      for (uint32_t ti = h; ti-- > 0;) do_tile(std::true_type{}, ti);
+    }
 #pragma unroll
     for (int g = 0; g < G; g++) {
-      if (S.item[g].type == 1 && S.item[g].size > 1) {
+      if (U.kind[g] == kWbCoded) {
         uint32_t* bitbuf = S.bitbuf[warp][g];
         if (lane == 0) bitbuf[(st[g].B - 32 * st[g].flushed) >> 5] |= 1u << (st[g].B & 31);
         __syncwarp();
         const uint32_t first_byte = max(4 * st[g].flushed, st[g].a);
-        const uint32_t end_byte = st[g].a + S.item[g].sbytes[s];
+        const uint32_t end_byte = st[g].a + U.sbytes[g];
         for (uint32_t bb = first_byte + lane; bb < end_byte; bb += 32) {
           const uint32_t rel = bb - 4 * st[g].flushed;
           st[g].gaddr[bb - st[g].a] = (uint8_t)(bitbuf[rel >> 2] >> (8 * (rel & 3)));
@@ -941,8 +1115,65 @@
         __syncwarp();
       }
     }
-  }
-}
+    ph.mark(kPhTail);
+    wb_cp_async_wait();
+    __syncwarp();
+    ph.mark(kPhSetup);
+    u = u_next;
+    b ^= 1;
+  }
+  ph.commit(lane);
+}
+
+#ifdef ZB_EMIT_PHASES
+template <int G>
+__global__ void __launch_bounds__(kWbWarps * 32) k_emit_ceiling(const uint8_t* __restrict__ in, uint64_t n, uint32_t chunk, uint64_t K,
+                                                                const uint32_t* __restrict__ sizes, const uint64_t* __restrict__ item_off,
+                                                                uint8_t* out, uint32_t* claim) {
+  const int lane = threadIdx.x & 31;
+  const uint64_t units = 4 * K;
+  for (;;) {
+    uint32_t v = 0;
+    if (lane == 0) v = atomicAdd(claim, 1u);
+    const uint64_t u = __shfl_sync(0xffffffffu, v, 0);
+    if (u >= units) break;
+    const uint64_t c = u >> 2;
+    const uint32_t s = (uint32_t)(u & 3);
+    const uint32_t chunk_len = (c == K - 1) ? (uint32_t)(n - c * (uint64_t)chunk) : chunk;
+    if (chunk_len % (64u * G) != 0) continue;
+    const uint32_t seg = chunk_len / G / 4;
+    const uint8_t* src = in + c * (uint64_t)chunk + (uint64_t)s * seg * G;
+    uint4* dst[G];
+    uint32_t per_tile[G];
+#pragma unroll
+    for (int g = 0; g < G; g++) {
+      const uint64_t item = (uint64_t)g * K + c;
+      const uint32_t q = sizes[item] / 4;
+      dst[g] = reinterpret_cast<uint4*>((reinterpret_cast<uintptr_t>(out + item_off[item] + (uint64_t)s * q) + 15) & ~(uintptr_t)15);
+      per_tile[g] = (q / 16) * kWbTile / seg;
+    }
+    const uint32_t ntiles = (seg + kWbTile - 1) / kWbTile;
+    uint4 cur[G], nxt[G];
+    {
+      const uint32_t t0 = (ntiles - 1) * kWbTile;
+      if (t0 + 16 * lane < seg)
+#pragma unroll
+        for (int i = 0; i < G; i++) nxt[i] = __ldg(reinterpret_cast<const uint4*>(src + (uint64_t)(t0 + 16 * lane) * G) + i);
+    }
+    for (uint32_t ti = ntiles; ti-- > 0;) {
+#pragma unroll
+      for (int i = 0; i < G; i++) cur[i] = nxt[i];
+      if (ti > 0)
+#pragma unroll
+        for (int i = 0; i < G; i++) nxt[i] = __ldg(reinterpret_cast<const uint4*>(src + (uint64_t)((ti - 1) * kWbTile + 16 * lane) * G) + i);
+      const uint32_t k = ntiles - 1 - ti;
+#pragma unroll
+      for (int g = 0; g < G; g++)
+        if ((uint32_t)lane < per_tile[g]) dst[g][k * per_tile[g] + lane] = cur[g];
+    }
+  }
+}
+#endif
 
 template <int G>
 __global__ void __launch_bounds__(kTableWarps * 32) k_encode_table_batch(EncBatch B) {
@@ -966,7 +1197,7 @@
     if (threadIdx.x == 0) T.ctrl->total_len = T.hdr_len;
     return;
   }
-  encode_scan_block(T.sizes, T.types, T.G, T.K, T.hdr, T.hdr_len, T.out, T.item_off, T.ctrl, T.partials,
+  encode_scan_block(T.sizes, T.types, T.saves, T.G, T.K, T.hdr, T.hdr_len, T.out, T.item_off, T.ctrl, T.partials,
                     (uint32_t)(blockIdx.x - B.start[i]));
 }
 
```

Result: no change. 547.4, median of 6 (+0.5%).
